# kpham-augment/LongLive

Measured on AMD Instinct MI355X. Metric: generated frames/sec (832x480) LongLive-1.3B, frame-sink + short-window attention, 4 denoise steps + clean-context pass, higher is better.
Workload: dtype bf16

## Files before the change

### include/longlive_hip.h

```cpp
#ifndef LONGLIVE_HIP_H
#define LONGLIVE_HIP_H

#include <stdint.h>

#ifdef __cplusplus
extern "C" {
#endif

typedef uint16_t ll_bf16;
typedef void* ll_stream;

enum ll_status {
  LL_OK = 0,
  LL_ERR_INVALID_ARG = -1,
  LL_ERR_LAUNCH = -2,
  LL_ERR_UNSUPPORTED = -3
};

enum ll_epilogue {
  LL_EPI_BIAS = 0,
  LL_EPI_BIAS_GELU = 1,
  LL_EPI_BIAS_GATE_RES = 2,
  LL_EPI_BIAS_RES = 3
};
// ... 68 lines not shown
               const ll_bf16* mod, int nmod, int gate_idx, int rows_per_batch, int frame_len, ll_stream stream);
int ll_gemm_mx_qkv(const uint8_t* xq, const uint8_t* sx, const uint8_t* wq, const uint8_t* sw, const ll_bf16* bias, ll_bf16* out,
                   int M, int N, int K, int ldo, ll_bf16* cache_v, int B, int L, int S, int write_start, int roped_offset,
                   int write_len, ll_stream stream);
int ll_ln_modulate_mx(const ll_bf16* x, uint8_t* q, uint8_t* qs, const ll_bf16* e, const ll_bf16* mod, int nmod, int shift_idx,
                      int scale_idx, int B, int L, int C, int F, float eps, ll_stream stream);
int ll_ln_modulate_tab_mx(const ll_bf16* x, uint8_t* q, uint8_t* qs, const float* tab, int nmod, int shift_idx, int scale_idx,
                          int B, int L, int C, int F, float eps, ll_stream stream);
int ll_layernorm_affine_mx(const ll_bf16* x, const ll_bf16* w, const ll_bf16* b, uint8_t* q, uint8_t* qs, int rows, int C,
                           float eps, ll_stream stream);
int ll_gemm_plan_mx(int M, int N, int K, char* out, int cap);

int ll_quantize_mx6(const ll_bf16* x, uint8_t* q, uint8_t* qs, int rows, int K, int ldx, ll_stream stream);
int ll_gemm_mx6(const uint8_t* xq, const uint8_t* sx, const uint8_t* wq, const uint8_t* sw, const ll_bf16* bias, ll_bf16* out,
                uint8_t* q_out, uint8_t* s_out, int M, int N, int K, int ldo, int epilogue, const ll_bf16* res, const ll_bf16* e,
                const ll_bf16* mod, int nmod, int gate_idx, int rows_per_batch, int frame_len, ll_stream stream);
int ll_gemm_mx6_qkv(const uint8_t* xq, const uint8_t* sx, const uint8_t* wq, const uint8_t* sw, const ll_bf16* bias, ll_bf16* out,
                    int M, int N, int K, int ldo, ll_bf16* cache_v, int B, int L, int S, int write_start, int roped_offset,
                    int write_len, ll_stream stream);
int ll_ln_modulate_mx6(const ll_bf16* x, uint8_t* q, uint8_t* qs, const ll_bf16* e, const ll_bf16* mod, int nmod, int shift_idx,
                       int scale_idx, int B, int L, int C, int F, float eps, ll_stream stream);
int ll_ln_modulate_tab_mx6(const ll_bf16* x, uint8_t* q, uint8_t* qs, const float* tab, int nmod, int shift_idx, int scale_idx,
                           int B, int L, int C, int F, float eps, ll_stream stream);
int ll_layernorm_affine_mx6(const ll_bf16* x, const ll_bf16* w, const ll_bf16* b, uint8_t* q, uint8_t* qs, int rows, int C,
                            float eps, ll_stream stream);
int ll_gemm_plan_mx6(int M, int N, int K, char* out, int cap);

int ll_quantize_mx4(const ll_bf16* x, uint8_t* q, uint8_t* qs, int rows, int K, int ldx, ll_stream stream);
int ll_gemm_mx4w6(const uint8_t* xq, const uint8_t* sx, const uint8_t* wq, const uint8_t* sw, const ll_bf16* bias, ll_bf16* out,
                  uint8_t* q_out, uint8_t* s_out, int M, int N, int K, int ldo, int epilogue, const ll_bf16* res, const ll_bf16* e,
                  const ll_bf16* mod, int nmod, int gate_idx, int rows_per_batch, int frame_len, ll_stream stream);
int ll_gemm_mx4w6_qkv(const uint8_t* xq, const uint8_t* sx, const uint8_t* wq, const uint8_t* sw, const ll_bf16* bias, ll_bf16* out,
                      int M, int N, int K, int ldo, ll_bf16* cache_v, int B, int L, int S, int write_start, int roped_offset,
                      int write_len, ll_stream stream);
int ll_gemm_plan_mx4w6(int M, int N, int K, char* out, int cap);

int ll_gemm_mx4(const uint8_t* xq, const uint8_t* sx, const uint8_t* wq, const uint8_t* sw, const ll_bf16* bias, ll_bf16* out,
                uint8_t* q_out, uint8_t* s_out, int M, int N, int K, int ldo, int epilogue, const ll_bf16* res, const ll_bf16* e,
                const ll_bf16* mod, int nmod, int gate_idx, int rows_per_batch, int frame_len, ll_stream stream);
int ll_gemm_mx4_qkv(const uint8_t* xq, const uint8_t* sx, const uint8_t* wq, const uint8_t* sw, const ll_bf16* bias, ll_bf16* out,
                    int M, int N, int K, int ldo, ll_bf16* cache_v, int B, int L, int S, int write_start, int roped_offset,
                    int write_len, ll_stream stream);
int ll_ln_modulate_mx4(const ll_bf16* x, uint8_t* q, uint8_t* qs, const ll_bf16* e, const ll_bf16* mod, int nmod, int shift_idx,
                       int scale_idx, int B, int L, int C, int F, float eps, ll_stream stream);
int ll_ln_modulate_tab_mx4(const ll_bf16* x, uint8_t* q, uint8_t* qs, const float* tab, int nmod, int shift_idx, int scale_idx,
                           int B, int L, int C, int F, float eps, ll_stream stream);
int ll_layernorm_affine_mx4(const ll_bf16* x, const ll_bf16* w, const ll_bf16* b, uint8_t* q, uint8_t* qs, int rows, int C,
                            float eps, ll_stream stream);
int ll_gemm_plan_mx4(int M, int N, int K, char* out, int cap);

int ll_quantize_rows_f8(const ll_bf16* x, uint8_t* q, float* scale, int rows, int K, int ldx, ll_stream stream);
int ll_gemm_f8(const uint8_t* xq, const float* sx, const uint8_t* wq, const float* sw, const ll_bf16* bias, ll_bf16* out,
               int M, int N, int K, int ldo, int epilogue, const ll_bf16* res, const ll_bf16* e, const ll_bf16* mod,
               int nmod, int gate_idx, int rows_per_batch, int frame_len, ll_stream stream);
int ll_gemm_f8_qkv(const uint8_t* xq, const float* sx, const uint8_t* wq, const float* sw, const ll_bf16* bias, ll_bf16* out,
                   int M, int N, int K, int ldo, ll_bf16* cache_v, int B, int L, int S, int write_start, int roped_offset,
                   int write_len, ll_stream stream);
int ll_ln_modulate_f8(const ll_bf16* x, uint8_t* q, float* qscale, const ll_bf16* e, const ll_bf16* mod, int nmod, int shift_idx,
                      int scale_idx, int B, int L, int C, int F, float eps, ll_stream stream);
int ll_ln_modulate_tab_f8(const ll_bf16* x, uint8_t* q, float* qscale, const float* tab, int nmod, int shift_idx, int scale_idx,
                          int B, int L, int C, int F, float eps, ll_stream stream);
int ll_layernorm_affine_f8(const ll_bf16* x, const ll_bf16* w, const ll_bf16* b, uint8_t* q, float* qscale, int rows, int C,
                           float eps, ll_stream stream);
int ll_gemm_plan_f8(int M, int N, int K, char* out, int cap);

int ll_kv_shadow_mx(const ll_bf16* k, const ll_bf16* v, uint8_t* kq, uint8_t* ks, uint8_t* vq, uint8_t* vs, int B, int S, int S32, int H,
                    int head_dim, int lo, int hi, ll_stream stream);
int ll_flash_attn_mx(const ll_bf16* q, const uint8_t* kq, const uint8_t* ks, const uint8_t* vq, const uint8_t* vs, ll_bf16* out, int B,
                     int Lq, int H, int head_dim, int ldq, int ldo, int S, int S32, int seg0_start, int seg0_len, int seg1_start,
                     int seg1_len, float scale, ll_stream stream);
int ll_flash_attn_mx_plan(int Lq, int H, int B, int seg0_start, int seg0_len, int seg1_start, int seg1_len, char* out, int cap);

int ll_linear_small(const ll_bf16* x, const ll_bf16* w, const ll_bf16* bias, ll_bf16* out, int M, int N, int K,
                    int act_in, int act_out, ll_stream stream);

int ll_flash_attn(const ll_bf16* q, const ll_bf16* k, const ll_bf16* v, ll_bf16* out, int B, int Lq, int H, int ldq,
                  int ldo, int ldk, long long k_batch_stride, int seg0_start, int seg0_len, int seg1_start,
                  int seg1_len, float scale, ll_stream stream);

int ll_gemm_ssq_planes(int M, int N, int K);
int ll_gemm_bf16_ssq(const ll_bf16* x, const ll_bf16* w, const ll_bf16* bias, ll_bf16* out, float* ssq, int M, int N, int K, int ldx,
                     int ldo, ll_stream stream);
int ll_flash_attn_qnorm_ok(int H, int nkeys);
int ll_flash_attn_qnorm(const ll_bf16* q, const float* ssq, const ll_bf16* norm_w, float eps, const ll_bf16* k, const ll_bf16* v,
                        ll_bf16* out, int B, int Lq, int H, int ldq, int ldo, int ldk, long long k_batch_stride, int key_start,
                        int nkeys, float scale, ll_stream stream);


int ll_patchify(const ll_bf16* x, ll_bf16* patches, int B, int F, int Cin, int H, int W, ll_stream stream);

int ll_sinusoid(const float* t, ll_bf16* out, int n, int dim, ll_stream stream);

int ll_unpatchify_x0(const ll_bf16* head, const ll_bf16* xt, const float* sigma, ll_bf16* flow, ll_bf16* x0, int B,
                     int F, int Cout, int H, int W, ll_stream stream);

int ll_add_noise(const ll_bf16* x0, const ll_bf16* noise, const float* sigma, ll_bf16* out, int N, long long inner,
                 ll_stream stream);

int ll_sigma_lookup(const float* t, const float* timesteps, const float* sigmas, float* out, int n, int n_table,
                    ll_stream stream);

int ll_synth_hash(float* out, long long lo, long long n, unsigned long long stream_const, int kind, ll_stream stream);


int ll_conv_cl(const ll_bf16* x, const ll_bf16* zero16, const ll_bf16* w, const ll_bf16* bias, const ll_bf16* res,
               ll_bf16* out, int T, int H, int W, int Cin, int Cout, int Kpad, int KT, int KH, int upsample, int ldo,
               ll_stream stream);
int ll_conv_cl_rms_ok(int H, int W, int Cin, int Cout, int KT, int KH, int upsample);
int ll_conv_cl_rms(const ll_bf16* x, const ll_bf16* zero16, const ll_bf16* w, const ll_bf16* bias, const ll_bf16* res, ll_bf16* out,
                   const ll_bf16* rms_gamma, ll_bf16* out_rms, int rms_silu, int T, int H, int W, int Cin, int Cout, int Kpad, int KT,
                   int KH, int upsample, int ldo, ll_stream stream);

int ll_rms_silu_cl(const ll_bf16* x, const ll_bf16* gamma, ll_bf16* out, long long pixels, int C, int do_silu,
                   ll_stream stream);

int ll_softmax_rows(const ll_bf16* s, ll_bf16* p, int rows, int N, int ld, float scale, ll_stream stream);

int ll_vae_unscale_cl(const ll_bf16* z, const ll_bf16* mean, const ll_bf16* inv_std, ll_bf16* out, int T, int C, int h,
                      int w, ll_stream stream);

int ll_cl_to_tchw_clamp(const ll_bf16* x, float* out, int T, int H, int W, int ldc, ll_stream stream);


int ll_t5_rmsnorm(const ll_bf16* x, const ll_bf16* w, ll_bf16* out, int rows, int C, float eps, ll_stream stream);

int ll_t5_gated_gelu(const ll_bf16* h, ll_bf16* out, long long M, int F, ll_stream stream);

int ll_gather_rows(const ll_bf16* table, const long long* ids, ll_bf16* out, int n, int C, long long vocab, ll_stream stream);

int ll_t5_attention(const ll_bf16* q, const ll_bf16* k, const ll_bf16* vt, const ll_bf16* bias_tab, ll_bf16* out, int L,
                    int H, int ldqk, int ldo, int seq_len, ll_stream stream);

#ifdef __cplusplus
}
#endif
#endif
```

### longlive_amd/_lib.py

```python
from __future__ import annotations

import ctypes as C
import os

_HERE = os.path.dirname(os.path.abspath(__file__))
LIB_PATH = os.path.join(_HERE, "liblonglive_hip.so")

ABI_VERSION = 111

_p, _i, _f, _ll = C.c_void_p, C.c_int, C.c_float, C.c_longlong

SIGNATURES = {
    "ll_version": [],
    "ll_last_error": [],
    "ll_set_tuning": [C.c_char_p, _i],
    "ll_gemm_plan": [_i, _i, _i, _i, C.c_char_p, _i],
    "ll_gemm_plan_epi": [_i, _i, _i, _i, _i, _i, C.c_char_p, _i],
    "ll_flash_attn_plan": [_i, _i, _i, _i, _i, _i, C.c_char_p, _i],
    "ll_ln_modulate": [_p, _p, _p, _p, _i, _i, _i, _i, _i, _i, _i, _f, _p],
    "ll_modulation_table": [_p, _p, _p, _i, _i, _i, _i, _p],
    "ll_modulation_table_f32": [_p, _p, _p, _i, _i, _i, _i, C.c_uint, _p],
    "ll_ln_modulate_tab": [_p, _p, _p, _p, _p, _i, _i, _i, _i, _i, _i, _i, _f, _p],
    "ll_layernorm_affine": [_p, _p, _p, _p, _i, _i, _f, _p],
    "ll_ln_modulate_q8": [_p, _p, _p, _p, _p, _i, _i, _i, _i, _i, _i, _i, _f, _p],
    "ll_layernorm_affine_q8": [_p, _p, _p, _p, _p, _i, _i, _f, _p],
    "ll_rmsnorm": [_p, _p, _p, _i, _i, _i, _i, _f, _p],
    "ll_qk_norm_rope_kv_store": [_p, _p, _p, _p, _p, _p, _p, _p, _i, _i, _i, _i, _i, _i, _i, _i, _i, _i, _f, _p],
    "ll_kv_roll": [_p, _p, _i, _i, _i, _i, _i, _i, _p],
    "ll_gemm_bf16": [_p, _p, _p, _p, _i, _i, _i, _i, _i, _i, _p, _p, _p, _i, _i, _i, _i, _p],
    "ll_gemm_ksplit_plan": [_i, _i, _i],
    "ll_gemm_ksplit_workspace_bytes": [_i, _i, _i],
    "ll_gemm_bf16_ksplit": [_p, _p, _p, _p, _i, _i, _i, _i, _i, _i, _p, _p, _ll, _p],
    "ll_gemm_bf16_ksplit_t5norm": [_p, _p, _p, _p, _i, _i, _i, _i, _i, _p, _p, _f, _p, _p, _ll, _p],
    "ll_gemm_w8a8": [_p, _p, _p, _p, _p, _p, _i, _i, _i, _i, _i, _p, _p, _p, _i, _i, _i, _i, _p],
    "ll_gemm_bf16_qkv": [_p, _p, _p, _p, _i, _i, _i, _i, _i, _p, _i, _i, _i, _i, _i, _i, _p],
    "ll_gemm_w8a8_qkv": [_p, _p, _p, _p, _p, _p, _i, _i, _i, _i, _p, _i, _i, _i, _i, _i, _i, _p],
    "ll_quantize_rows": [_p, _p, _p, _i, _i, _i, _p],
    "ll_linear_small": [_p, _p, _p, _p, _i, _i, _i, _i, _i, _p],
    "ll_flash_attn": [_p, _p, _p, _p, _i, _i, _i, _i, _i, _i, _ll, _i, _i, _i, _i, _f, _p],
    "ll_patchify": [_p, _p, _i, _i, _i, _i, _i, _p],
    "ll_sinusoid": [_p, _p, _i, _i, _p],
    "ll_unpatchify_x0": [_p, _p, _p, _p, _p, _i, _i, _i, _i, _i, _p],
    "ll_add_noise": [_p, _p, _p, _p, _i, _ll, _p],
    "ll_sigma_lookup": [_p, _p, _p, _p, _i, _i, _p],
    "ll_synth_hash": [_p, _ll, _ll, C.c_ulonglong, _i, _p],
    "ll_gemm_ssq_planes": [_i, _i, _i],
    "ll_gemm_bf16_ssq": [_p, _p, _p, _p, _p, _i, _i, _i, _i, _i, _p],
    "ll_flash_attn_qnorm_ok": [_i, _i],
    "ll_flash_attn_qnorm": [_p, _p, _p, _f, _p, _p, _p, _i, _i, _i, _i, _i, _i, _ll, _i, _i, _f, _p],
    "ll_conv_cl": [_p] * 6 + [_i] * 10 + [_p],
    "ll_conv_cl_rms_ok": [_i] * 7,
    "ll_conv_cl_rms": [_p] * 8 + [_i] * 11 + [_p],
    "ll_rms_silu_cl": [_p, _p, _p, _ll, _i, _i, _p],
    "ll_softmax_rows": [_p, _p, _i, _i, _i, _f, _p],
    "ll_vae_unscale_cl": [_p, _p, _p, _p, _i, _i, _i, _i, _p],
    "ll_cl_to_tchw_clamp": [_p, _p, _i, _i, _i, _i, _p],
    "ll_t5_rmsnorm": [_p, _p, _p, _i, _i, _f, _p],
    "ll_t5_gated_gelu": [_p, _p, _ll, _i, _p],
    "ll_gather_rows": [_p, _p, _p, _i, _i, _ll, _p],
    "ll_t5_attention": [_p, _p, _p, _p, _p, _i, _i, _i, _i, _i, _p],
    "ll_quantize_mx": [_p, _p, _p, _i, _i, _i, _p],
    "ll_gemm_mx": [_p, _p, _p, _p, _p, _p, _p, _p, _i, _i, _i, _i, _i, _p, _p, _p, _i, _i, _i, _i, _p],
    "ll_gemm_mx_qkv": [_p, _p, _p, _p, _p, _p, _i, _i, _i, _i, _p, _i, _i, _i, _i, _i, _i, _p],
    "ll_ln_modulate_mx": [_p, _p, _p, _p, _p, _i, _i, _i, _i, _i, _i, _i, _f, _p],
    "ll_ln_modulate_tab_mx": [_p, _p, _p, _p, _i, _i, _i, _i, _i, _i, _i, _f, _p],
    "ll_layernorm_affine_mx": [_p, _p, _p, _p, _p, _i, _i, _f, _p],
    "ll_gemm_plan_mx": [_i, _i, _i, C.c_char_p, _i],
    "ll_kv_shadow_mx": [_p] * 6 + [_i] * 7 + [_p],
    "ll_flash_attn_mx": [_p] * 6 + [_i] * 12 + [_f, _p],
    "ll_flash_attn_mx_plan": [_i] * 7 + [C.c_char_p, _i],
    "ll_quantize_rows_f8": [_p, _p, _p, _i, _i, _i, _p],
    "ll_gemm_f8": [_p, _p, _p, _p, _p, _p, _i, _i, _i, _i, _i, _p, _p, _p, _i, _i, _i, _i, _p],
    "ll_gemm_f8_qkv": [_p, _p, _p, _p, _p, _p, _i, _i, _i, _i, _p, _i, _i, _i, _i, _i, _i, _p],
    "ll_ln_modulate_f8": [_p, _p, _p, _p, _p, _i, _i, _i, _i, _i, _i, _i, _f, _p],
    "ll_ln_modulate_tab_f8": [_p, _p, _p, _p, _i, _i, _i, _i, _i, _i, _i, _f, _p],
    "ll_layernorm_affine_f8": [_p, _p, _p, _p, _p, _i, _i, _f, _p],
    "ll_gemm_plan_f8": [_i, _i, _i, C.c_char_p, _i],
    "ll_quantize_mx6": [_p, _p, _p, _i, _i, _i, _p],
    "ll_gemm_mx6": [_p] * 8 + [_i] * 5 + [_p] * 3 + [_i] * 4 + [_p],
    "ll_gemm_mx6_qkv": [_p] * 6 + [_i] * 4 + [_p] + [_i] * 6 + [_p],
    "ll_ln_modulate_mx6": [_p] * 5 + [_i] * 7 + [_f, _p],
    "ll_ln_modulate_tab_mx6": [_p] * 4 + [_i] * 7 + [_f, _p],
    "ll_layernorm_affine_mx6": [_p] * 5 + [_i, _i, _f, _p],
    "ll_gemm_plan_mx6": [_i, _i, _i, C.c_char_p, _i],
    "ll_quantize_mx4": [_p, _p, _p, _i, _i, _i, _p],
    "ll_gemm_mx4w6": [_p] * 8 + [_i] * 5 + [_p] * 3 + [_i] * 4 + [_p],
    "ll_gemm_mx4w6_qkv": [_p] * 6 + [_i] * 4 + [_p] + [_i] * 6 + [_p],
    "ll_gemm_plan_mx4w6": [_i, _i, _i, C.c_char_p, _i],
    "ll_gemm_mx4": [_p] * 8 + [_i] * 5 + [_p] * 3 + [_i] * 4 + [_p],
    "ll_gemm_mx4_qkv": [_p] * 6 + [_i] * 4 + [_p] + [_i] * 6 + [_p],
    "ll_ln_modulate_mx4": [_p] * 5 + [_i] * 7 + [_f, _p],
    "ll_ln_modulate_tab_mx4": [_p] * 4 + [_i] * 7 + [_f, _p],
    "ll_layernorm_affine_mx4": [_p] * 5 + [_i, _i, _f, _p],
    "ll_gemm_plan_mx4": [_i, _i, _i, C.c_char_p, _i],
}
_RESTYPES = {"ll_last_error": C.c_char_p, "ll_gemm_ksplit_workspace_bytes": C.c_longlong}

_lib = None


def load() -> C.CDLL:
    global _lib
    if _lib is not None:
        return _lib
    path = os.environ.get("LONGLIVE_HIP_LIB", LIB_PATH)
    if not os.path.exists(path):
        raise RuntimeError(
            f"{path} not found: the HIP extension is not built (make -C longlive_amd/csrc). "
            "longlive_amd has no CPU fallback by design.")
    lib = C.CDLL(path)
    for name, argtypes in SIGNATURES.items():
        try:
            fn = getattr(lib, name)
        except AttributeError as exc:
            raise RuntimeError(f"{LIB_PATH} does not export {name}") from exc
        fn.argtypes = argtypes
        fn.restype = _RESTYPES.get(name, C.c_int)
    if lib.ll_version() != ABI_VERSION:
        raise RuntimeError(f"{path} has ABI version {lib.ll_version()}, this binding needs {ABI_VERSION}: rebuild it "
                           "(make -C longlive_amd/csrc); a stale library would misread every argument list")
    _lib = lib
    for kv in filter(None, os.environ.get("LL_TUNING", "").split(",")):
        k, v = kv.split("=")
        if lib.ll_set_tuning(k.encode(), int(v)) != 0:
            raise RuntimeError(f"LL_TUNING: {lib.ll_last_error().decode()}")
    return lib


def check(rc: int, what: str = "") -> None:
    if rc != 0:
        msg = load().ll_last_error()
# ... 2 lines not shown
```

### longlive_amd/csrc/elementwise.hip

```cpp
#include "common.h"
#include "mx.h"
#include "mx4.h"
#include "mx6.h"

#define MAXCH 4

struct RowRegs {
  f32x2 p[MAXCH][4];
};
struct RowWords {
  unsigned w[MAXCH][4];
};

template <bool FULL>
__device__ __forceinline__ bool in_row(int c, int C) {
  return FULL || c < C;
}

template <int NCH, bool FULL>
__device__ __forceinline__ void load_words(const bf16* __restrict__ p, int C, int lane, RowWords& r) {
#pragma unroll
  for (int i = 0; i < NCH; ++i) {
    int c = (lane + 64 * i) * 8;
    uint4 t = make_uint4(0u, 0u, 0u, 0u);
// ... 866 lines not shown

#define DISPATCH_NCH(C, CALL)                                              \
  do {                                                                     \
    int nch_ = ((C) + 511) / 512;                                          \
    bool full_ = ((C) % 512) == 0;                                         \
    if (nch_ == 1) { if (full_) CALL(1, true); else CALL(1, false); }      \
    else if (nch_ == 2) { if (full_) CALL(2, true); else CALL(2, false); } \
    else if (nch_ == 3) { if (full_) CALL(3, true); else CALL(3, false); } \
    else { if (full_) CALL(4, true); else CALL(4, false); }                \
  } while (0)

static inline bool row_ok(int C) { return C > 0 && C <= 2048 && (C % 8) == 0; }

static int ln_modulate_launch(const ll_bf16* x, ll_bf16* out, int8_t* q, float* qscale, const ll_bf16* e,
                              const ll_bf16* mod, int nmod, int shift_idx, int scale_idx, int B, int L, int C, int F,
                              float eps, ll_stream stream, bool f8 = false) {
  LL_REQUIRE(row_ok(C), "ll_ln_modulate: C=%d must be a multiple of 8 and <= 2048", C);
  LL_REQUIRE(F > 0 && L % F == 0, "ll_ln_modulate: L=%d not divisible by F=%d", L, F);
  LL_REQUIRE(shift_idx >= 0 && shift_idx < nmod && scale_idx >= 0 && scale_idx < nmod, "ll_ln_modulate: bad mod index");
  int rows = B * L;
  if (rows == 0) return LL_OK;
  dim3 grid((rows + 3) / 4);
#define CALL2(N, FL, F8)                                                                                                     \
  do {                                                                                                                   \
    if (mod)                                                                                                             \
      hipLaunchKernelGGL((ln_modulate_kernel<N, FL, false, F8>), grid, dim3(256), 0, (hipStream_t)stream, (const bf16*)x, (bf16*)out, \
                         (const bf16*)e, (const bf16*)mod, nmod, shift_idx, scale_idx, rows, L, C, L / F, F, eps, q, qscale); \
    else                                                                                                                 \
      hipLaunchKernelGGL((ln_modulate_kernel<N, FL, true, F8>), grid, dim3(256), 0, (hipStream_t)stream, (const bf16*)x, (bf16*)out,  \
                         (const bf16*)e, (const bf16*)mod, nmod, shift_idx, scale_idx, rows, L, C, L / F, F, eps, q, qscale); \
  } while (0)
#define CALL(N, FL) CALL2(N, FL, false)
#define CALL_F8(N, FL) CALL2(N, FL, true)
  if (f8) DISPATCH_NCH(C, CALL_F8);
  else DISPATCH_NCH(C, CALL);
#undef CALL
#undef CALL_F8
#undef CALL2
  return ll_check_launch("ll_ln_modulate");
}

extern "C" int ll_modulation_table(const ll_bf16* e, const ll_bf16* mods, ll_bf16* out, int num_layers, int BF, int nmod, int C,
                                   ll_stream stream) {
  LL_REQUIRE(C > 0 && C % 8 == 0 && nmod > 0 && num_layers >= 0 && BF >= 0, "ll_modulation_table: bad shape");
  long long chunks = (long long)num_layers * BF * nmod * (C / 8);
  if (chunks == 0) return LL_OK;
  LL_REQUIRE(chunks < (1LL << 31) * 256, "ll_modulation_table: too large");
  hipLaunchKernelGGL(modulation_table_kernel, dim3((unsigned)((chunks + 255) / 256)), dim3(256), 0, (hipStream_t)stream,
                     (const bf16*)e, (const bf16*)mods, (bf16*)out, num_layers, BF, nmod * (C / 8));
  return ll_check_launch("ll_modulation_table");
}

extern "C" int ll_ln_modulate(const ll_bf16* x, ll_bf16* out, const ll_bf16* e, const ll_bf16* mod, int nmod,
                              int shift_idx, int scale_idx, int B, int L, int C, int F, float eps, ll_stream stream) {
  return ln_modulate_launch(x, out, nullptr, nullptr, e, mod, nmod, shift_idx, scale_idx, B, L, C, F, eps, stream);
}

extern "C" int ll_ln_modulate_q8(const ll_bf16* x, int8_t* q, float* qscale, const ll_bf16* e, const ll_bf16* mod,
                                 int nmod, int shift_idx, int scale_idx, int B, int L, int C, int F, float eps,
                                 ll_stream stream) {
  LL_REQUIRE(q && qscale, "ll_ln_modulate_q8: q and qscale are required");
  return ln_modulate_launch(x, nullptr, q, qscale, e, mod, nmod, shift_idx, scale_idx, B, L, C, F, eps, stream);
}

extern "C" int ll_ln_modulate_f8(const ll_bf16* x, uint8_t* q, float* qscale, const ll_bf16* e, const ll_bf16* mod, int nmod,
                                 int shift_idx, int scale_idx, int B, int L, int C, int F, float eps, ll_stream stream) {
  LL_REQUIRE(x != nullptr && e != nullptr, "ll_ln_modulate_f8: x and e are required");
  LL_REQUIRE(q && qscale, "ll_ln_modulate_f8: codes and scales are required");
  return ln_modulate_launch(x, nullptr, (int8_t*)q, qscale, e, mod, nmod, shift_idx, scale_idx, B, L, C, F, eps, stream, true);
}

extern "C" int ll_modulation_table_f32(const ll_bf16* e, const ll_bf16* mods, float* out, int num_layers, int BF, int nmod, int C,
                                       unsigned one_plus_mask, ll_stream stream) {
  LL_REQUIRE(C > 0 && C % 8 == 0 && nmod > 0 && nmod <= 32 && num_layers >= 0 && BF >= 0, "ll_modulation_table_f32: bad shape");
  LL_REQUIRE(nmod == 32 || (one_plus_mask >> nmod) == 0, "ll_modulation_table_f32: one_plus_mask names a chunk >= nmod=%d", nmod);
  long long chunks = (long long)num_layers * BF * nmod * (C / 8);
  if (chunks == 0) return LL_OK;
  LL_REQUIRE(chunks < (1LL << 31) * 256, "ll_modulation_table_f32: too large");
  hipLaunchKernelGGL(modulation_table_f32_kernel, dim3((unsigned)((chunks + 255) / 256)), dim3(256), 0, (hipStream_t)stream,
                     (const bf16*)e, (const bf16*)mods, out, num_layers, BF, nmod, C / 8, one_plus_mask);
  return ll_check_launch("ll_modulation_table_f32");
}

extern "C" int ll_ln_modulate_tab(const ll_bf16* x, ll_bf16* out, int8_t* q, float* qscale, const float* tab, int nmod,
                                  int shift_idx, int scale_idx, int B, int L, int C, int F, float eps, ll_stream stream) {
  LL_REQUIRE(row_ok(C), "ll_ln_modulate_tab: C=%d must be a multiple of 8 and <= 2048", C);
  LL_REQUIRE(F > 0 && L % F == 0, "ll_ln_modulate_tab: L=%d not divisible by F=%d", L, F);
  LL_REQUIRE(shift_idx >= 0 && shift_idx < nmod && scale_idx >= 0 && scale_idx < nmod, "ll_ln_modulate_tab: bad mod index");
  LL_REQUIRE((out != nullptr) != (q != nullptr), "ll_ln_modulate_tab: exactly one of out (bf16) and q (int8, with qscale) is required");
  LL_REQUIRE(q == nullptr || qscale != nullptr, "ll_ln_modulate_tab: q needs qscale");
  int rows = B * L;
  if (rows == 0) return LL_OK;
  dim3 grid((rows + 3) / 4);
#define CALL(N, FL)                                                                                                      \
  hipLaunchKernelGGL((ln_modulate_tab_kernel<N, FL>), grid, dim3(256), 0, (hipStream_t)stream, (const bf16*)x, (bf16*)out, tab, \
                     nmod, shift_idx, scale_idx, rows, L, C, L / F, F, eps, q, qscale)
  DISPATCH_NCH(C, CALL);
#undef CALL
  return ll_check_launch("ll_ln_modulate_tab");
}

extern "C" int ll_ln_modulate_tab_f8(const ll_bf16* x, uint8_t* q, float* qscale, const float* tab, int nmod, int shift_idx, int scale_idx,
                                     int B, int L, int C, int F, float eps, ll_stream stream) {
  LL_REQUIRE(x != nullptr && tab != nullptr, "ll_ln_modulate_tab_f8: x and tab are required");
  LL_REQUIRE(q && qscale, "ll_ln_modulate_tab_f8: codes and scales are required");
  LL_REQUIRE(row_ok(C), "ll_ln_modulate_tab_f8: C=%d must be a multiple of 8 and <= 2048", C);
  LL_REQUIRE(F > 0 && L % F == 0, "ll_ln_modulate_tab_f8: L=%d not divisible by F=%d", L, F);
  LL_REQUIRE(shift_idx >= 0 && shift_idx < nmod && scale_idx >= 0 && scale_idx < nmod, "ll_ln_modulate_tab_f8: bad mod index");
  int rows = B * L;
  if (rows == 0) return LL_OK;
  dim3 grid((rows + 3) / 4);
#define CALL(N, FL)                                                                                                           \
  hipLaunchKernelGGL((ln_modulate_tab_kernel<N, FL, true>), grid, dim3(256), 0, (hipStream_t)stream, (const bf16*)x, (bf16*)nullptr, \
                     tab, nmod, shift_idx, scale_idx, rows, L, C, L / F, F, eps, (int8_t*)q, qscale)
  DISPATCH_NCH(C, CALL);
#undef CALL
  return ll_check_launch("ll_ln_modulate_tab_f8");
}

static int layernorm_affine_launch(const ll_bf16* x, const ll_bf16* w, const ll_bf16* b, ll_bf16* out, int8_t* q,
                                   float* qscale, int rows, int C, float eps, ll_stream stream, bool f8 = false) {
  LL_REQUIRE(row_ok(C), "ll_layernorm_affine: C=%d must be a multiple of 8 and <= 2048", C);
  if (rows == 0) return LL_OK;
  dim3 grid((rows + 3) / 4);
#define CALL2(N, FL, F8)                                                                                         \
  hipLaunchKernelGGL((layernorm_affine_kernel<N, FL, F8>), grid, dim3(256), 0, (hipStream_t)stream, (const bf16*)x, \
                     (const bf16*)w, (const bf16*)b, (bf16*)out, rows, C, eps, q, qscale)
#define CALL(N, FL) CALL2(N, FL, false)
#define CALL_F8(N, FL) CALL2(N, FL, true)
  if (f8) DISPATCH_NCH(C, CALL_F8);
  else DISPATCH_NCH(C, CALL);
#undef CALL
#undef CALL_F8
#undef CALL2
  return ll_check_launch("ll_layernorm_affine");
}

extern "C" int ll_layernorm_affine(const ll_bf16* x, const ll_bf16* w, const ll_bf16* b, ll_bf16* out, int rows, int C,
                                   float eps, ll_stream stream) {
  return layernorm_affine_launch(x, w, b, out, nullptr, nullptr, rows, C, eps, stream);
}

extern "C" int ll_layernorm_affine_q8(const ll_bf16* x, const ll_bf16* w, const ll_bf16* b, int8_t* q, float* qscale,
                                      int rows, int C, float eps, ll_stream stream) {
  LL_REQUIRE(q && qscale, "ll_layernorm_affine_q8: q and qscale are required");
  return layernorm_affine_launch(x, w, b, nullptr, q, qscale, rows, C, eps, stream);
}

extern "C" int ll_layernorm_affine_f8(const ll_bf16* x, const ll_bf16* w, const ll_bf16* b, uint8_t* q, float* qscale, int rows, int C,
                                      float eps, ll_stream stream) {
  LL_REQUIRE(x != nullptr && w != nullptr && b != nullptr, "ll_layernorm_affine_f8: x, w and b are required");
  LL_REQUIRE(q && qscale, "ll_layernorm_affine_f8: codes and scales are required");
  return layernorm_affine_launch(x, w, b, nullptr, (int8_t*)q, qscale, rows, C, eps, stream, true);
}

static int mx_row_ok(const char* fn, int C, const void* q, const void* qs) {
  LL_REQUIRE(C > 0 && C <= 2048 && C % MX_BLOCK == 0, "%s: C=%d must be a multiple of 32 and <= 2048", fn, C);
  LL_REQUIRE(q != nullptr && qs != nullptr, "%s: codes and scales are required", fn);
  return LL_OK;
}

extern "C" int ll_ln_modulate_mx(const ll_bf16* x, uint8_t* q, uint8_t* qs, const ll_bf16* e, const ll_bf16* mod, int nmod,
                                 int shift_idx, int scale_idx, int B, int L, int C, int F, float eps, ll_stream stream) {
  if (int rc = mx_row_ok("ll_ln_modulate_mx", C, q, qs)) return rc;
  LL_REQUIRE(x != nullptr && e != nullptr, "ll_ln_modulate_mx: x and e are required");
  LL_REQUIRE(F > 0 && L % F == 0, "ll_ln_modulate_mx: L=%d not divisible by F=%d", L, F);
// ... 294 lines not shown
```

### longlive_amd/csrc/gemm.hip

```cpp
#include <stdio.h>
#include <string.h>
#include <atomic>

#include "gemm_common.h"
#include "mx.h"

#define V2_BM 256
#define V2_STAGE ((V2_BM + BN) * ROWB)

template <int EPI, int Q>
__global__ __launch_bounds__(512, 2) void gemm_kernel_v2(const char* __restrict__ X, const char* __restrict__ Wt,
                                                         bf16* __restrict__ Y, int M, int N, int nk, size_t xrow_bytes,
                                                         size_t wrow_bytes, int ldo, int ntm, int ntn, int gm, int lds_epi, EpiArgs ea) {
  extern __shared__ __attribute__((aligned(16))) char smem[];
  typedef typename Ty<Q>::frag frag_t;
  const int tid = threadIdx.x, lane = tid & 63;
  const int wave = __builtin_amdgcn_readfirstlane(tid >> 6);
  const int wm = wave >> 1, wn = wave & 1;
  int lid = xcd_remap(blockIdx.x, ntm * ntn), mt_, nt_;
  tile_of(lid, ntm, ntn, gm, mt_, nt_);
  const int m0 = mt_ * V2_BM, n0 = nt_ * BN;

  typename Ty<Q>::acc acc[4][4];
#pragma unroll
// ... 490 lines not shown
    if (v5 || v6) {                                                                                                    \
      (void)ll_lds_attr((const void*)gemm_kernel_v5<E, Q, 2, 4, 8, 3>, 2 * (256 + 192) * ROWB);                       \
      (void)ll_lds_attr((const void*)gemm_kernel_v5<E, Q, 4, 2, 4, 7>, 2 * (256 + 224) * ROWB);                       \
      if (v5)                                                                                                          \
        hipLaunchKernelGGL((gemm_kernel_v5<E, Q, 2, 4, 8, 3>), grid, block, lds, s, (const char*)x, (const char*)w, out, M, N, nk, \
                           xrow_bytes, wrow_bytes, ldo, ntm, ntn, gm, lds_epi, ea);                                                 \
      else                                                                                                             \
        hipLaunchKernelGGL((gemm_kernel_v5<E, Q, 4, 2, 4, 7>), grid, block, lds, s, (const char*)x, (const char*)w, out, M, N, nk, \
                           xrow_bytes, wrow_bytes, ldo, ntm, ntn, gm, lds_epi, ea);                                                 \
    } else if (v3) {                                                                                                   \
      (void)ll_lds_attr((const void*)gemm_kernel_v3<E, Q>, (int)lds);                                                 \
      hipLaunchKernelGGL((gemm_kernel_v3<E, Q>), grid, block, lds, s, (const char*)x, (const char*)w, out, M, N, nk,   \
                         xrow_bytes, wrow_bytes, ldo, ntm, ntn, gm, lds_epi, ea);                                      \
    } else {                                                                                                           \
      (void)ll_lds_attr((const void*)gemm_kernel_v2<E, Q>, (int)lds);                                          \
      hipLaunchKernelGGL((gemm_kernel_v2<E, Q>), grid, block, lds, s, (const char*)x, (const char*)w, out, M, N, nk, \
                         xrow_bytes, wrow_bytes, ldo, ntm, ntn, gm, lds_epi, ea);                                      \
    }                                                                                                                  \
  } while (0)
  switch (epilogue) {
    case LL_EPI_BIAS: LAUNCH(LL_EPI_BIAS); break;
    case LL_EPI_BIAS_GELU: LAUNCH(LL_EPI_BIAS_GELU); break;
    case LL_EPI_BIAS_GATE_RES: LAUNCH(LL_EPI_BIAS_GATE_RES); break;
    default: LAUNCH(LL_EPI_BIAS_RES); break;
  }
#undef LAUNCH
  return LL_OK;
}

static int check_epilogue(const char* fn, int M, int N, int ldo, int epilogue, const void* bias, const void* res,
                          const void* e, const void* mod, int nmod, int gate_idx, int rows_per_batch, int frame_len) {
  LL_REQUIRE(N > 0 && N % 8 == 0, "%s: N=%d must be a positive multiple of 8", fn, N);
  LL_REQUIRE(ldo >= N && ldo % 4 == 0, "%s: ldo=%d must be >= N and a multiple of 4", fn, ldo);
  LL_REQUIRE(bias != nullptr, "%s: bias is required", fn);
  LL_REQUIRE(epilogue >= 0 && epilogue <= 3, "%s: unknown epilogue %d", fn, epilogue);
  if (epilogue == LL_EPI_BIAS_GATE_RES) {
    LL_REQUIRE(res && e, "%s: gate-residual epilogue needs res and e (mod may be NULL: e then holds bf16(mod + e))", fn);
    LL_REQUIRE(frame_len > 0 && rows_per_batch > 0 && rows_per_batch % frame_len == 0 && M % rows_per_batch == 0,
               "%s: rows_per_batch=%d / frame_len=%d do not tile M=%d", fn, rows_per_batch, frame_len, M);
    LL_REQUIRE(gate_idx >= 0 && gate_idx < nmod, "%s: gate_idx %d outside nmod %d", fn, gate_idx, nmod);
  }
  if (epilogue == LL_EPI_BIAS_RES) LL_REQUIRE(res != nullptr, "%s: residual epilogue needs res", fn);
  return LL_OK;
}

extern "C" int ll_gemm_bf16(const ll_bf16* x, const ll_bf16* w, const ll_bf16* bias, ll_bf16* out, int M, int N, int K,
                            int ldx, int ldo, int epilogue, const ll_bf16* res, const ll_bf16* e, const ll_bf16* mod,
                            int nmod, int gate_idx, int rows_per_batch, int frame_len, ll_stream stream) {
  LL_REQUIRE(K > 0 && K % 64 == 0, "ll_gemm_bf16: K=%d must be a positive multiple of 64", K);
  LL_REQUIRE(ldx >= K && ldx % 8 == 0, "ll_gemm_bf16: ldx=%d must be >= K and a multiple of 8", ldx);
  int rc = check_epilogue("ll_gemm_bf16", M, N, ldo, epilogue, bias, res, e, mod, nmod, gate_idx, rows_per_batch, frame_len);
  if (rc) return rc;
  if (M == 0) return LL_OK;
  EpiArgs ea{(const bf16*)bias, (const bf16*)res, (const bf16*)e, (const bf16*)mod, nullptr, nullptr, nmod, gate_idx,
             rows_per_batch, frame_len, frame_len > 0 && rows_per_batch > 0 ? rows_per_batch / frame_len : 0};
  if (int lrc = launch_gemm<GQ_BF16>(x, w, (bf16*)out, M, N, K, (size_t)ldx * 2, (size_t)K * 2, ldo, epilogue, ea, (hipStream_t)stream)) return lrc;
  return ll_check_launch("ll_gemm_bf16");
}

static int device_cus();
int gemm_asm_ssq_launch(const bf16* x, const bf16* w, const bf16* bias, bf16* out, float* ssq, int M, int N, int K, int ldx, int ldo, int gm,
                        hipStream_t s);
extern "C" int ll_gemm_ssq_planes(int M, int N, int K) {
  if (!gemm_asm_wanted(LL_EPI_BIAS)) return 0;
  return gemm_asm_width(M, N, K, K, LL_EPI_BIAS, true, false, false, 0) == 128 && N / 128 <= 16 ? N / 128 : 0;
}
extern "C" int ll_gemm_bf16_ssq(const ll_bf16* x, const ll_bf16* w, const ll_bf16* bias, ll_bf16* out, float* ssq, int M, int N, int K,
                                int ldx, int ldo, ll_stream stream) {
  LL_REQUIRE(K > 0 && K % 64 == 0, "ll_gemm_bf16_ssq: K=%d must be a positive multiple of 64", K);
  LL_REQUIRE(ldx >= K && ldx % 8 == 0, "ll_gemm_bf16_ssq: ldx=%d must be >= K and a multiple of 8", ldx);
  int rc = check_epilogue("ll_gemm_bf16_ssq", M, N, ldo, LL_EPI_BIAS, bias, nullptr, nullptr, nullptr, 0, 0, 0, 0);
  if (rc) return rc;
  LL_REQUIRE(ssq != nullptr && ((size_t)ssq & 3) == 0, "ll_gemm_bf16_ssq: ssq is required");
  LL_REQUIRE(ll_gemm_ssq_planes(M, N, K) > 0 && ldx == K, "ll_gemm_bf16_ssq: %d x %d x %d is not covered by the generated kernel under the current "
             "tuning (ask ll_gemm_ssq_planes first and run ll_gemm_bf16 + ll_rmsnorm instead)", M, N, K);
  if (M == 0) return LL_OK;
  const int r = gemm_asm_ssq_launch((const bf16*)x, (const bf16*)w, (const bf16*)bias, (bf16*)out, ssq, M, N, K, ldx, ldo, g_gemm_group_m,
                                    (hipStream_t)stream);
  if (r < 0) return r;
  LL_REQUIRE(r == 1, "ll_gemm_bf16_ssq: the generated kernel refused a shape its plan accepted");
  return ll_check_launch("ll_gemm_bf16_ssq");
}

extern "C" int ll_gemm_ksplit_plan(int M, int N, int K) {
  if (!gemm_asm_wanted(LL_EPI_BIAS)) return 0;
  return gemm_ksplit_splits(M, N, K, device_cus());
}
extern "C" long long ll_gemm_ksplit_workspace_bytes(int M, int N, int K) {
  const int S = ll_gemm_ksplit_plan(M, N, K);
  return S ? (long long)S * M * N * 4 : 0;
}
extern "C" int ll_gemm_bf16_ksplit(const ll_bf16* x, const ll_bf16* w, const ll_bf16* bias, ll_bf16* out, int M, int N, int K,
                                   int ldx, int ldo, int epilogue, const ll_bf16* res, void* workspace,
                                   long long workspace_bytes, ll_stream stream) {
  LL_REQUIRE(K > 0 && K % 64 == 0, "ll_gemm_bf16_ksplit: K=%d must be a positive multiple of 64", K);
  LL_REQUIRE(ldx >= K && ldx % 8 == 0, "ll_gemm_bf16_ksplit: ldx=%d must be >= K and a multiple of 8", ldx);
  LL_REQUIRE(epilogue == LL_EPI_BIAS || epilogue == LL_EPI_BIAS_RES, "ll_gemm_bf16_ksplit: epilogue %d (bias or bias + residual only)", epilogue);
  int rc = check_epilogue("ll_gemm_bf16_ksplit", M, N, ldo, epilogue, bias, res, nullptr, nullptr, 0, 0, 0, 0);
  if (rc) return rc;
  LL_REQUIRE(workspace_bytes >= 0 && (workspace != nullptr || workspace_bytes == 0), "ll_gemm_bf16_ksplit: workspace_bytes without a workspace");
  if (M == 0) return LL_OK;
  const int S = ll_gemm_ksplit_plan(M, N, K);
  if (S >= 2 && workspace != nullptr && ldo % 8 == 0) {
    LL_REQUIRE(workspace_bytes >= (long long)S * M * N * 4 && ((size_t)workspace & 15) == 0,
               "ll_gemm_bf16_ksplit: workspace of %lld bytes, need %lld (16-byte aligned)", workspace_bytes, (long long)S * M * N * 4);
    const int r = gemm_asm_ksplit_launch((const bf16*)x, (const bf16*)w, (const bf16*)bias, (bf16*)out, M, N, K, ldx, ldo, epilogue,
                                         (const bf16*)res, (float*)workspace, S, g_gemm_group_m, (hipStream_t)stream, nullptr, 0.f, nullptr);
    if (r) return r < 0 ? r : ll_check_launch("ll_gemm_bf16_ksplit");
  }
  EpiArgs ea{(const bf16*)bias, (const bf16*)res, nullptr, nullptr, nullptr, nullptr, 0, 0, 0, 0, 0};
  if (int lrc = launch_gemm<GQ_BF16>(x, w, (bf16*)out, M, N, K, (size_t)ldx * 2, (size_t)K * 2, ldo, epilogue, ea, (hipStream_t)stream)) return lrc;
  return ll_check_launch("ll_gemm_bf16_ksplit");
}

extern "C" int ll_gemm_bf16_ksplit_t5norm(const ll_bf16* x, const ll_bf16* w, const ll_bf16* bias, ll_bf16* out, int M, int N, int K,
                                          int ldx, int ldo, const ll_bf16* res, const ll_bf16* norm_w, float eps, ll_bf16* h_out,
                                          void* workspace, long long workspace_bytes, ll_stream stream) {
  LL_REQUIRE(K > 0 && K % 64 == 0, "ll_gemm_bf16_ksplit_t5norm: K=%d must be a positive multiple of 64", K);
  LL_REQUIRE(ldx >= K && ldx % 8 == 0, "ll_gemm_bf16_ksplit_t5norm: ldx=%d must be >= K and a multiple of 8", ldx);
  LL_REQUIRE(norm_w != nullptr && h_out != nullptr, "ll_gemm_bf16_ksplit_t5norm: needs the norm weight and an output for the normalised rows");
  LL_REQUIRE(ldo == N, "ll_gemm_bf16_ksplit_t5norm: ldo=%d must equal N=%d (the norm runs over whole rows)", ldo, N);
  int rc = check_epilogue("ll_gemm_bf16_ksplit_t5norm", M, N, ldo, LL_EPI_BIAS_RES, bias, res, nullptr, nullptr, 0, 0, 0, 0);
  if (rc) return rc;
  LL_REQUIRE(workspace_bytes >= 0 && (workspace != nullptr || workspace_bytes == 0), "ll_gemm_bf16_ksplit_t5norm: workspace_bytes without a workspace");
  if (M == 0) return LL_OK;
  const int S = ll_gemm_ksplit_plan(M, N, K);
  if (S >= 2 && workspace != nullptr && N <= 4096) {
    LL_REQUIRE(workspace_bytes >= (long long)S * M * N * 4 && ((size_t)workspace & 15) == 0,
               "ll_gemm_bf16_ksplit_t5norm: workspace of %lld bytes, need %lld (16-byte aligned)", workspace_bytes, (long long)S * M * N * 4);
    const int r = gemm_asm_ksplit_launch((const bf16*)x, (const bf16*)w, (const bf16*)bias, (bf16*)out, M, N, K, ldx, ldo, LL_EPI_BIAS_RES,
                                         (const bf16*)res, (float*)workspace, S, g_gemm_group_m, (hipStream_t)stream, (const bf16*)norm_w, eps,
                                         (bf16*)h_out);
    if (r) return r < 0 ? r : ll_check_launch("ll_gemm_bf16_ksplit_t5norm");
  }
  rc = ll_gemm_bf16_ksplit(x, w, bias, out, M, N, K, ldx, ldo, LL_EPI_BIAS_RES, res, workspace, workspace_bytes, stream);
  if (rc) return rc;
  return ll_t5_rmsnorm(out, norm_w, h_out, M, N, eps, stream);
}

static int device_cus() {
  static int cus[64];
  int dev = 0;
  if (hipGetDevice(&dev) != hipSuccess || dev < 0 || dev >= 64) return 0;
  if (cus[dev] == 0) {
    int n = 0;
    if (hipDeviceGetAttribute(&n, hipDeviceAttributeMultiprocessorCount, dev) != hipSuccess) n = 0;
    cus[dev] = n > 0 ? n : -1;
  }
  return cus[dev] > 0 ? cus[dev] : 0;
}

extern "C" int ll_gemm_plan_epi(int M, int N, int K, int int8, int epilogue, int plain, char* out, int cap) {
  LL_REQUIRE(out != nullptr && cap > 0, "ll_gemm_plan_epi: needs an output buffer");
  if (!int8 && gemm_asm_wanted(epilogue)) {
    const int wn = gemm_asm_width(M, N, K, K, epilogue, plain != 0, plain == 2, plain == 2 && (2 * (N / 3)) % 192 == 0, 1);
    if (wn) { gemm_asm_plan(M, N, wn, epilogue, out, cap, false); ll_plan_append_knobs(out, cap); return LL_OK; }
  }
  if (int8 && (g_gemm_asm & 16) && gemm_asm_wanted(epilogue)) {
    const int wn = gemm_asm_width_i8(M, N, K, epilogue, plain != 0, plain == 2, plain == 2 && (2 * (N / 3)) % 192 == 0, 1);
    if (wn) { gemm_asm_plan(M, N, wn, epilogue, out, cap, true); ll_plan_append_knobs(out, cap); return LL_OK; }
  }
  return ll_gemm_plan(M, N, K, int8, out, cap);
}

extern "C" int ll_gemm_w8a8(const int8_t* xq, const float* sx, const int8_t* wq, const float* sw, const ll_bf16* bias,
                            ll_bf16* out, int M, int N, int K, int ldo, int epilogue, const ll_bf16* res,
// ... 134 lines not shown
```

### longlive_amd/csrc/gemm_asm.hip

```cpp
#include "gemm_common.h"

#define GA_NAME gemm_asm_224_gelu
#define GA_WN 224
#define GA_INC "build/gemm_asm_224_1.inc"
#include "gemm_asm_kernel.inl"
#undef GA_NAME
#undef GA_WN
#undef GA_INC
#define GA_NAME gemm_asm_256_bias
#define GA_WN 256
#define GA_INC "build/gemm_asm_256_0.inc"
#include "gemm_asm_kernel.inl"
#undef GA_NAME
#undef GA_WN
#undef GA_INC
#define GA_NAME gemm_asm_192_bias
#define GA_WN 192
#define GA_INC "build/gemm_asm_192_0.inc"
#include "gemm_asm_kernel.inl"
#undef GA_NAME
#undef GA_WN
#undef GA_INC
#define GA_NAME gemm_asm_128_bias
#define GA_WN 128
#define GA_INC "build/gemm_asm_128_0.inc"
#include "gemm_asm_kernel.inl"
#undef GA_NAME
#undef GA_WN
#undef GA_INC
#define GA_NAME gemm_asm_128_gate_res
#define GA_WN 128
#define GA_INC "build/gemm_asm_128_2.inc"
#include "gemm_asm_kernel.inl"
#undef GA_NAME
#undef GA_WN
#undef GA_INC
#define GA_NAME gemm_asm_128_res
#define GA_WN 128
#define GA_INC "build/gemm_asm_128_3.inc"
#include "gemm_asm_kernel.inl"
#undef GA_NAME
#undef GA_WN
#undef GA_INC

#define GA_NAME gemm_asmp_224_gelu
#define GA_INC "build/gemm_asmp_224_1.inc"
#include "gemm_asm_kernel_p.inl"
#undef GA_NAME
#undef GA_INC
#define GA_NAME gemm_asmp_192_bias
#define GA_INC "build/gemm_asmp_192_0.inc"
#include "gemm_asm_kernel_p.inl"
#undef GA_NAME
#undef GA_INC
#define GA_NAME gemm_asmp_128_bias
#define GA_INC "build/gemm_asmp_128_0.inc"
#include "gemm_asm_kernel_p.inl"
#undef GA_NAME
#undef GA_INC
#define GA_NAME gemm_asmp_128_gate_res
#define GA_INC "build/gemm_asmp_128_2.inc"
#include "gemm_asm_kernel_p.inl"
#undef GA_NAME
#undef GA_INC
#define GA_NAME gemm_asmp_128_res
#define GA_INC "build/gemm_asmp_128_3.inc"
#include "gemm_asm_kernel_p.inl"
#undef GA_NAME
#undef GA_INC

#define GA_NAME gemm_asm_128_bias_ssq
#define GA_WN 128
#define GA_INC "build/gemm_asm_128_5.inc"
#define GA_SSQ 1
#include "gemm_asm_kernel.inl"
#undef GA_SSQ
#undef GA_NAME
#undef GA_WN
#undef GA_INC

#define GA_NAME gemm_asm_128_partial
#define GA_WN 128
#define GA_INC "build/gemm_asm_128_4.inc"
#define GA_PARTIAL 1
#include "gemm_asm_kernel.inl"
#undef GA_PARTIAL
#undef GA_NAME
#undef GA_WN
#undef GA_INC

#define GA_NAME gemm_asmq_224_gelu
#define GA_WN 224
#define GA_INC "build/gemm_asmq_224_1.inc"
#define GA_I8 1
#include "gemm_asm_kernel.inl"
#undef GA_I8
#undef GA_NAME
#undef GA_WN
#undef GA_INC
#define GA_NAME gemm_asmq_192_bias
#define GA_WN 192
#define GA_INC "build/gemm_asmq_192_0.inc"
#define GA_I8 1
#include "gemm_asm_kernel.inl"
#undef GA_I8
#undef GA_NAME
#undef GA_WN
#undef GA_INC
#define GA_NAME gemm_asmq_128_bias
#define GA_WN 128
#define GA_INC "build/gemm_asmq_128_0.inc"
#define GA_I8 1
#include "gemm_asm_kernel.inl"
#undef GA_I8
#undef GA_NAME
#undef GA_WN
#undef GA_INC
#define GA_NAME gemm_asmq_128_gate_res
#define GA_WN 128
#define GA_INC "build/gemm_asmq_128_2.inc"
#define GA_I8 1
#include "gemm_asm_kernel.inl"
#undef GA_I8
#undef GA_NAME
#undef GA_WN
#undef GA_INC
#define GA_NAME gemm_asmq_128_res
#define GA_WN 128
#define GA_INC "build/gemm_asmq_128_3.inc"
#define GA_I8 1
#include "gemm_asm_kernel.inl"
#undef GA_I8
#undef GA_NAME
#undef GA_WN
#undef GA_INC

int g_gemm_asm_persistent = 1;
static int gemm_asm_cus() {
  static int cus[64];
  int dev = 0;
  if (hipGetDevice(&dev) != hipSuccess || dev < 0 || dev >= 64) return 0;
  if (cus[dev] == 0) {
    int n = 0;
    if (hipDeviceGetAttribute(&n, hipDeviceAttributeMultiprocessorCount, dev) != hipSuccess) n = 0;
    cus[dev] = n > 0 ? n : -1;
  }
  return cus[dev] > 0 ? cus[dev] : 0;
}

int gemm_asm_width(int M, int N, int K, int ldx, int epilogue, bool plain, bool has_v, bool v_ok, int frame_len) {
  if (!plain || M <= 0 || K % 64 != 0 || K < 256 || (ldx % 8) != 0) return 0;
  if (epilogue == LL_EPI_BIAS_GATE_RES && frame_len <= 0) return 0;
  if ((long long)256 * ldx * 2 >= 0x7fffffffLL || (long long)256 * K * 2 >= 0x7fffffffLL) return 0;
  if (has_v) return (v_ok && epilogue == LL_EPI_BIAS && N % 192 == 0) ? 192 : 0;
  if (epilogue == LL_EPI_BIAS_GELU) return N % 224 == 0 ? 224 : 0;
  if (epilogue == LL_EPI_BIAS && N > 2048 && N % 192 == 0) return 192;
  if (epilogue == LL_EPI_BIAS && M <= 1024 && N >= 16384 && N % 256 == 0) return 256;
  if (N % 128 == 0 && (N <= 2048 || M <= 1024) &&
      (epilogue == LL_EPI_BIAS || epilogue == LL_EPI_BIAS_GATE_RES || epilogue == LL_EPI_BIAS_RES)) return 128;
  return 0;
}

int gemm_asm_launch(const bf16* x, const bf16* w, bf16* out, int M, int N, int K, int ldx, int ldo, int epilogue, const EpiArgs& ea,
                    int gm, hipStream_t s) {
  const bool has_v = ea.v_out != nullptr;
  const bool v_ok = has_v && ea.v_L == M && ea.v_col0 % 192 == 0 && ea.v_C > 0;
  const int wn = gemm_asm_width(M, N, K, ldx, epilogue, ea.sx == nullptr && ea.mod == nullptr, has_v, v_ok, ea.frame_len);
  if (!wn) return 0;
  const void* fn = wn == 224 ? (const void*)gemm_asm_224_gelu
                   : wn == 256 ? (const void*)gemm_asm_256_bias
                   : wn == 192 ? (const void*)gemm_asm_192_bias
                   : epilogue == LL_EPI_BIAS ? (const void*)gemm_asm_128_bias
                   : epilogue == LL_EPI_BIAS_GATE_RES ? (const void*)gemm_asm_128_gate_res : (const void*)gemm_asm_128_res;
  const int lds = 3 * wn * 128 + 4 * 2 * 8192;
  const int ntm = (M + 255) / 256, ntn = N / wn;
  const int cus = gemm_asm_cus() & ~7;
  const void* pfn = wn == 224 ? (const void*)gemm_asmp_224_gelu
                    : wn == 192 ? (const void*)gemm_asmp_192_bias
                    : wn != 128 ? nullptr
                    : epilogue == LL_EPI_BIAS ? (const void*)gemm_asmp_128_bias
                    : epilogue == LL_EPI_BIAS_GATE_RES ? (const void*)gemm_asmp_128_gate_res : (const void*)gemm_asmp_128_res;
  const bool persistent = g_gemm_asm_persistent && pfn != nullptr && cus >= 8 && ntm * ntn > cus;
  if (persistent) fn = pfn;
  if (int rc = ll_lds_attr(fn, lds)) return rc;
  const bf16* gate = epilogue == LL_EPI_BIAS_GATE_RES ? ea.e + (size_t)ea.gate_idx * N : nullptr;
  const int gstride = ea.nmod * N * 2;
  bf16* v_out = ea.v_out;
  int v_col0 = ea.v_col0, v_C = ea.v_C, v_shift = ea.v_write_start - ea.v_roped_offset, v_lo = ea.v_roped_offset,
      v_hi = ea.v_roped_offset + ea.v_write_len;
  void* args[] = {(void*)&x, (void*)&w, (void*)&ea.bias, (void*)&out, (void*)&ea.res, (void*)&gate, (void*)&M, (void*)&N, (void*)&K,
                  (void*)&ldx, (void*)&ldo, (void*)&ea.frame_len, (void*)&gstride, (void*)&ntm, (void*)&ntn, (void*)&gm,
                  (void*)&v_out, (void*)&v_col0, (void*)&v_C, (void*)&v_shift, (void*)&v_lo, (void*)&v_hi};
  if (hipLaunchKernel(fn, dim3(persistent ? cus : ntm * ntn), dim3(256), args, (size_t)lds, s) != hipSuccess) return ll_check_launch("gemm_asm");
  return 1;
}

int gemm_asm_ssq_launch(const bf16* x, const bf16* w, const bf16* bias, bf16* out, float* ssq, int M, int N, int K, int ldx, int ldo, int gm,
                        hipStream_t s) {
  if (gemm_asm_width(M, N, K, ldx, LL_EPI_BIAS, true, false, false, 0) != 128) return 0;
  const void* fn = (const void*)gemm_asm_128_bias_ssq;
  const int lds = 3 * 128 * 128 + 4 * 2 * 8192;
  if (int rc = ll_lds_attr(fn, lds)) return rc;
  const int ntm = (M + 255) / 256, ntn = N / 128;
  const bf16* nullb = nullptr;
  bf16* nov = nullptr;
  int zero = 0;
  void* args[] = {(void*)&x, (void*)&w, (void*)&bias, (void*)&out, (void*)&nullb, (void*)&nullb, (void*)&M, (void*)&N, (void*)&K,
                  (void*)&ldx, (void*)&ldo, (void*)&zero, (void*)&zero, (void*)&ntm, (void*)&ntn, (void*)&gm,
                  (void*)&nov, (void*)&zero, (void*)&zero, (void*)&zero, (void*)&zero, (void*)&zero, (void*)&ssq};
  if (hipLaunchKernel(fn, dim3(ntm * ntn), dim3(256), args, (size_t)lds, s) != hipSuccess) return ll_check_launch("gemm_asm_128_bias_ssq");
  return 1;
}

const char* gemm_asm_plan(int M, int N, int wn, int epilogue, char* out, int cap, bool i8) {
  const char* tail = wn == 224 ? "gelu" : wn == 256 ? "bias" : epilogue == LL_EPI_BIAS ? "bias" : epilogue == LL_EPI_BIAS_GATE_RES ? "gate_res" : "res";
  const int tiles = ((M + 255) / 256) * (N / wn), cus = gemm_asm_cus() & ~7;
  if (!i8 && g_gemm_asm_persistent && wn != 256 && cus >= 8 && tiles > cus)
    snprintf(out, (size_t)cap, "gemm_asmp_%d_%s<bf16> tile 256x%d (4 waves x 64 rows, one wave per SIMD, generated schedule), %d persistent workgroups "
             "walk %d tiles, next tile staged under the epilogue", wn, tail, wn, cus, tiles);
  else
    snprintf(out, (size_t)cap, "gemm_asm%s_%d_%s<%s> tile 256x%d (4 waves x 64 rows, one wave per SIMD, generated schedule), %d workgroups", i8 ? "q" : "", wn,
             tail, i8 ? "i8" : "bf16", wn, tiles);
  return out;
}

int gemm_asm_width_i8(int M, int N, int K, int epilogue, bool plain, bool has_v, bool v_ok, int frame_len) {
  if (!plain || M <= 0 || K % 128 != 0 || K < 512 || (long long)256 * K >= 0x7fffffffLL) return 0;
  if (epilogue == LL_EPI_BIAS_GATE_RES && frame_len <= 0) return 0;
  if (has_v) return (v_ok && epilogue == LL_EPI_BIAS && N % 192 == 0) ? 192 : 0;
  if (epilogue == LL_EPI_BIAS_GELU) return N % 224 == 0 ? 224 : 0;
  if (epilogue == LL_EPI_BIAS && N > 2048 && N % 192 == 0) return 192;
  if (N % 128 == 0 && N <= 2048) return 128;
  return 0;
}

template <int EPI>
__global__ __launch_bounds__(256) void gemm_ksplit_reduce_kernel(const float* __restrict__ part, int splits, int M, int N,
                                                                 const bf16* __restrict__ bias, const bf16* __restrict__ res,
                                                                 bf16* __restrict__ out, int ldo) {
  const int n8 = N / 8;
  const long long idx = (long long)blockIdx.x * 256 + threadIdx.x;
  if (idx >= (long long)M * n8) return;
  const int m = (int)(idx / n8), n = (int)(idx - (long long)m * n8) * 8;
  float acc[8];
#pragma unroll
  for (int j = 0; j < 8; ++j) acc[j] = 0.f;
  for (int s = 0; s < splits; ++s) {
    const float4* p = reinterpret_cast<const float4*>(part + ((size_t)s * M + m) * N + n);
    float4 a = p[0], b = p[1];
    acc[0] += a.x; acc[1] += a.y; acc[2] += a.z; acc[3] += a.w; acc[4] += b.x; acc[5] += b.y; acc[6] += b.z; acc[7] += b.w;
  }
  bf16x8 bv = *reinterpret_cast<const bf16x8*>(bias + n), o;
  bf16x8 rv;
  if (EPI == LL_EPI_BIAS_RES) rv = *reinterpret_cast<const bf16x8*>(res + (size_t)m * ldo + n);
#pragma unroll
  for (int j = 0; j < 8; ++j) {
    bf16 v = (bf16)(acc[j] + (float)bv[j]);
    o[j] = EPI == LL_EPI_BIAS_RES ? (bf16)((float)rv[j] + (float)v) : v;
  }
  *reinterpret_cast<bf16x8*>(out + (size_t)m * ldo + n) = o;
}

__global__ __launch_bounds__(256) void gemm_ksplit_reduce_norm_kernel(const float* __restrict__ part, int splits, int M, int N,
                                                                      const bf16* __restrict__ bias, const bf16* __restrict__ res,
                                                                      bf16* __restrict__ out, int ldo, const bf16* __restrict__ nw,
                                                                      float eps, bf16* __restrict__ h_out) {
  __shared__ float sh[4];
  const int m = blockIdx.x;
  bf16x8 xn[2];
  float ss = 0.f;
#pragma unroll
  for (int i = 0; i < 2; ++i) {
    const int n = threadIdx.x * 8 + 2048 * i;
    if (n < N) {
      float acc[8];
#pragma unroll
      for (int j = 0; j < 8; ++j) acc[j] = 0.f;
      for (int s = 0; s < splits; ++s) {
        const float4* p = reinterpret_cast<const float4*>(part + ((size_t)s * M + m) * N + n);
        float4 a = p[0], b = p[1];
        acc[0] += a.x; acc[1] += a.y; acc[2] += a.z; acc[3] += a.w; acc[4] += b.x; acc[5] += b.y; acc[6] += b.z; acc[7] += b.w;
      }
      bf16x8 bv = *reinterpret_cast<const bf16x8*>(bias + n), rv = *reinterpret_cast<const bf16x8*>(res + (size_t)m * ldo + n), o;
#pragma unroll
      for (int j = 0; j < 8; ++j) {
        bf16 v = (bf16)(acc[j] + (float)bv[j]);
        o[j] = (bf16)((float)rv[j] + (float)v);
        ss += (float)o[j] * (float)o[j];
      }
      xn[i] = o;
      *reinterpret_cast<bf16x8*>(out + (size_t)m * ldo + n) = o;
    }
  }
  ss = t5_block_sum(ss, sh);
  const float r = rsqrtf(ss / (float)N + eps);
#pragma unroll
// ... 79 lines not shown
```

### longlive_amd/csrc/gen/gemm_asm_gen.py

```python
#!/usr/bin/env python3
from __future__ import annotations

import os
import sys

sys.path.insert(0, os.path.dirname(os.path.abspath(__file__)))
import attn_asm_gen as _A
from attn_asm_gen import Gen, finalize, lint, sreg, vreg, areg, to_inc, f32bits, spread

EPI_BIAS, EPI_GELU, EPI_GATE_RES, EPI_RES = 0, 1, 2, 3
EPI_PARTIAL = 4
EPI_BIAS_SSQ = 5

S_X, S_W, S_Y, S_BIAS, S_RES, S_GATE = 8, 10, 12, 14, 16, 18
S_LDX, S_LDW, S_LDO = 20, 21, 22
S_ROWS, S_COLS, S_NK = 23, 24, 25
S_FLEN, S_GSTRIDE, S_M0 = 26, 27, 28
S_ROWLO = 29
S_SX, S_SW = 64, 66
S_SSQ = 64
S_XRS, S_WRS = 32, 36
S_WAVE, S_I, S_T0, S_T1, S_T2 = 40, 41, 44, 45, 46
S_WM0, S_XK, S_WK, S_XKMAX, S_WKMAX = 47, 48, 49, 43, 62
S_MSK = 50
V_TID = 0

NSLOT, XU = 3, 2
S_XM0 = 30

S_XB, S_WB, S_YB, S_BIASB, S_RESB, S_GATEB = 84, 86, 88, 90, 92, 94
S_LDO0, S_MM, S_NN = 68, 69, 70
S_TILE, S_GRID, S_NTILES, S_NTM, S_NTN, S_GM = 71, 72, 73, 74, 75, 76
S_VHI, S_VOUT, S_VCOL0, S_VC2, S_VSHIFT, S_VLO = 77, 78, 80, 81, 82, 83
S_XN, S_WN, S_PF, S_ROWSN = 64, 66, 31, 42
S_MT, S_NT = 54, 55


def KN(k):
    return _A.knob_env("ASM_G_", k, 0)


class Cfg:
    def __init__(self, WN, epi, i8=False):
        assert WN % 32 == 0 and 64 <= WN <= 256
        assert not (i8 and epi in (EPI_PARTIAL, EPI_BIAS_SSQ))
        self.WN, self.NB, self.MB, self.epi, self.i8 = WN, WN // 32, 2, epi, i8
        self.nacc = self.MB * self.NB * 16
        self.slotb = WN * 128
        self.npw = WN // 32
        self.xbase = NSLOT * self.slotb
        self.xunit = 64 * 128
        self.lds_bytes = self.xbase + 4 * XU * self.xunit
        assert self.lds_bytes <= 160 * 1024
        self.FW = 0
        self.FX = 2 * self.NB * 2 * 4
        nxt = max(self.FX + 2 * self.MB * 4 * 4, 144)
        self.V_WOFF = nxt
        self.V_XROFF = nxt + 12
        self.V_DW = nxt + 16
        self.V_DX = nxt + 24
        self.V_LANE, self.V_R, self.V_H, self.V_ROW = nxt + 32, nxt + 33, nxt + 34, nxt + 35
        self.V_T = 0
        assert nxt + 37 <= 256, nxt
        self.V_EA = nxt + 37
        top = self.V_EA + 5
        if i8:
            self.V_SX = top + 2
            top += 6
        assert top % 2 == 0, top
        self.nl = {EPI_GATE_RES: 6, EPI_RES: 2}.get(epi, 0)
        self.V_E0 = top
        top += 16 if self.nl else 0
        self.V_SS = top
        top += 4 if epi == EPI_BIAS_SSQ else 0
        self.V_EB = top
        self.early_nb = 0 if epi == EPI_PARTIAL else max(0, min(self.NB, (256 - top) // 8))

    def acc(self, mb, nb):
        return (mb * self.NB + nb) * 16

    def fw(self, p, nb, ks):
        return self.FW + ((p * self.NB + nb) * 2 + ks) * 4

    def fx(self, b, mb, ks4):
        return self.FX + ((b * self.MB + mb) * 4 + ks4) * 4


def mfmas(c: Cfg, h):
    p, b, hf = h & 1, (h >> 1) & 1, h & 1
    out = []
    for ks in range(2):
        for nb in range(c.NB):
            for mb in range(c.MB):
                a = areg(c.acc(mb, nb), 16)
                op = "v_mfma_i32_32x32x32_i8" if c.i8 else "v_mfma_f32_32x32x16_bf16"
                out.append(f"{op} {a}, {vreg(c.fw(p, nb, ks), 4)}, {vreg(c.fx(b, mb, 2 * hf + ks), 4)}, {a}")
    return out


def w_frag_reads(c: Cfg, h):
    slot, hs = (h >> 1) % NSLOT, h & 1
    out = []
    for ks in range(2):
        for nb in range(c.NB):
            off = slot * c.slotb + nb * 4096
            b64, imm = off >> 16, off & 0xFFFF
            out.append(f"ds_read_b128 {vreg(c.fw(h & 1, nb, ks), 4)}, {vreg(c.V_WOFF + 4 * b64 + 2 * hs + ks)} offset:{imm}")
    return out


def x_frag_reads(c: Cfg, s):
    out = []
    for ks4 in range(4):
        for mb in range(c.MB):
            out.append(f"ds_read_b128 {vreg(c.fx(s & 1, mb, ks4), 4)}, {vreg(c.V_XROFF + ks4)} offset:{(s % XU) * c.xunit + mb * 4096}")
    return out


def x_dma(c: Cfg, s):
    out = []
    for i in range(8):
        out.append(f"s_add_u32 m0, {sreg(S_XM0)}, {(s % XU) * c.xunit + 1024 * i}")
        out.append(f"buffer_load_dwordx4 {vreg(c.V_DX + i)}, {sreg(S_XRS, 4)}, {sreg(S_XK)} offen lds")
    out.append(f"s_add_u32 {sreg(S_XK)}, {sreg(S_XK)}, 128")
    out.append(f"s_min_u32 {sreg(S_XK)}, {sreg(S_XK)}, {sreg(S_XKMAX)}")
    return out


def w_dma(c: Cfg, s):
    out = []
    for i in range(c.npw):
        out.append(f"s_add_u32 m0, {sreg(S_WM0)}, {(s % NSLOT) * c.slotb + 1024 * i}")
        out.append(f"buffer_load_dwordx4 {vreg(c.V_DW + i)}, {sreg(S_WRS, 4)}, {sreg(S_WK)} offen lds")
    out.append(f"s_add_u32 {sreg(S_WK)}, {sreg(S_WK)}, 128")
    out.append(f"s_min_u32 {sreg(S_WK)}, {sreg(S_WK)}, {sreg(S_WKMAX)}")
    return out


def drop_loads(ops):
    return [o for o in ops if not o.startswith("buffer_load")]


def udiv(g: Gen, q, num, den, T):
    I = g.I
    I(f"v_cvt_f32_u32 {vreg(T)}, {sreg(num)}")
    I(f"v_cvt_f32_u32 {vreg(T + 1)}, {sreg(den)}")
    I(f"v_rcp_f32 {vreg(T + 1)}, {vreg(T + 1)}")
    I("s_nop 0")
    I(f"v_mul_f32 {vreg(T)}, {vreg(T)}, {vreg(T + 1)}")
    I(f"v_cvt_u32_f32 {vreg(T)}, {vreg(T)}")
    I("s_nop 0")
    I(f"v_readfirstlane_b32 {sreg(q)}, {vreg(T)}")
    I("s_nop 0")
    I(f"s_mul_i32 {sreg(S_T2)}, {sreg(q)}, {sreg(den)}")
    I(f"s_cmp_gt_u32 {sreg(S_T2)}, {sreg(num)}")
    I(f"s_cselect_b32 {sreg(S_T2)}, 1, 0")
    I(f"s_sub_u32 {sreg(q)}, {sreg(q)}, {sreg(S_T2)}")
    I(f"s_mul_i32 {sreg(S_T2)}, {sreg(q)}, {sreg(den)}")
    I(f"s_sub_u32 {sreg(S_T2)}, {sreg(num)}, {sreg(S_T2)}")
# ... 11 lines not shown
    I(f"s_lshr_b32 {sreg(hi)}, {sreg(tile)}, 3")
    I(f"s_add_u32 {sreg(q1)}, {sreg(q)}, 1")
    I(f"s_mul_i32 {sreg(a)}, {sreg(x)}, {sreg(q1)}")
    I(f"s_mul_i32 {sreg(b)}, {sreg(r)}, {sreg(q1)}")
    I(f"s_sub_u32 {sreg(c_)}, {sreg(x)}, {sreg(r)}")
    I(f"s_mul_i32 {sreg(c_)}, {sreg(c_)}, {sreg(q)}")
    I(f"s_add_u32 {sreg(b)}, {sreg(b)}, {sreg(c_)}")
    I(f"s_cmp_lt_u32 {sreg(x)}, {sreg(r)}")
    I(f"s_cselect_b32 {sreg(a)}, {sreg(a)}, {sreg(b)}")
    I(f"s_add_u32 {sreg(S_T0)}, {sreg(a)}, {sreg(hi)}")
    I(f"s_mul_i32 {sreg(S_T1)}, {sreg(S_GM)}, {sreg(S_NTN)}")
    udiv(g, 56, S_T0, S_T1, T)
    I(f"s_mul_i32 {sreg(57)}, {sreg(56)}, {sreg(S_T1)}")
    I(f"s_sub_u32 {sreg(S_T0)}, {sreg(S_T0)}, {sreg(57)}")
    I(f"s_mul_i32 {sreg(58)}, {sreg(56)}, {sreg(S_GM)}")
    I(f"s_sub_u32 {sreg(S_T1)}, {sreg(S_NTM)}, {sreg(58)}")
    I(f"s_min_u32 {sreg(S_T1)}, {sreg(S_T1)}, {sreg(S_GM)}")
    udiv(g, S_NT, S_T0, S_T1, T)
    I(f"s_mul_i32 {sreg(57)}, {sreg(S_NT)}, {sreg(S_T1)}")
    I(f"s_sub_u32 {sreg(57)}, {sreg(S_T0)}, {sreg(57)}")
    I(f"s_add_u32 {sreg(S_MT)}, {sreg(58)}, {sreg(57)}")


def add64(g: Gen, dst, base, lo, hi=None):
    g.I(f"s_add_u32 {sreg(dst)}, {sreg(base)}, {sreg(lo)}")
    g.I(f"s_addc_u32 {sreg(dst + 1)}, {sreg(base + 1)}, {sreg(hi) if hi is not None else 0}")


def gen_tile_bases(g: Gen, c, xdst, wdst, rows_dst, skip_label, full: bool, prefix: str):
    I = g.I
    m0r, n0 = 56, 57
    I(f"s_lshl_b32 {sreg(m0r)}, {sreg(S_MT)}, 8")
    I(f"s_mul_i32 {sreg(n0)}, {sreg(S_NT)}, {c.WN}")
    I(f"s_mul_i32 {sreg(S_T0)}, {sreg(m0r)}, {sreg(S_LDX)}")
    I(f"s_mul_hi_u32 {sreg(S_T1)}, {sreg(m0r)}, {sreg(S_LDX)}")
    add64(g, xdst, S_XB, S_T0, S_T1)
    I(f"s_mul_i32 {sreg(S_T0)}, {sreg(n0)}, {sreg(S_LDW)}")
    I(f"s_mul_hi_u32 {sreg(S_T1)}, {sreg(n0)}, {sreg(S_LDW)}")
    add64(g, wdst, S_WB, S_T0, S_T1)
    I(f"s_sub_u32 {sreg(rows_dst)}, {sreg(S_MM)}, {sreg(m0r)}")
    if full:
        I(f"s_sub_u32 {sreg(S_COLS)}, {sreg(S_NN)}, {sreg(n0)}")
        I(f"s_mov_b32 {sreg(S_M0)}, {sreg(m0r)}")
        I(f"s_mov_b32 {sreg(S_ROWLO)}, 0")
        I(f"s_mov_b32 {sreg(S_LDO)}, {sreg(S_LDO0)}")
        I(f"s_lshl_b32 {sreg(58)}, {sreg(n0)}, 1")
        add64(g, S_BIAS, S_BIASB, 58)
        add64(g, S_GATE, S_GATEB, 58)
        I(f"s_mul_i32 {sreg(S_T0)}, {sreg(m0r)}, {sreg(S_LDO0)}")
        I(f"s_mul_hi_u32 {sreg(S_T1)}, {sreg(m0r)}, {sreg(S_LDO0)}")
        I(f"s_add_u32 {sreg(S_T0)}, {sreg(S_T0)}, {sreg(58)}")
        I(f"s_addc_u32 {sreg(S_T1)}, {sreg(S_T1)}, 0")
        add64(g, S_Y, S_YB, S_T0, S_T1)
        add64(g, S_RES, S_RESB, S_T0, S_T1)
    g.uid += 1
    lab = f"{prefix}_NOTV_{g.uid}"
    I(f"s_cmp_eq_u64 {sreg(S_VOUT, 2)}, 0")
    I(f"s_cbranch_scc1 {lab}")
    I(f"s_cmp_lt_u32 {sreg(n0)}, {sreg(S_VCOL0)}")
    I(f"s_cbranch_scc1 {lab}")
    I(f"s_min_i32 {sreg(59)}, {sreg(S_MM)}, {sreg(S_VHI)}")
    I(f"s_sub_i32 {sreg(59)}, {sreg(59)}, {sreg(m0r)}")
    I(f"s_sub_i32 {sreg(60)}, {sreg(S_VLO)}, {sreg(m0r)}")
    I(f"s_max_i32 {sreg(60)}, {sreg(60)}, 0")
    I(f"s_cmp_le_i32 {sreg(59)}, {sreg(60)}")
    I(f"s_cbranch_scc1 {skip_label}")
    I(f"s_mov_b32 {sreg(rows_dst)}, {sreg(59)}")
    if full:
        I(f"s_mov_b32 {sreg(S_ROWLO)}, {sreg(60)}")
        I(f"s_mov_b32 {sreg(S_LDO)}, {sreg(S_VC2)}")
        I(f"s_add_i32 {sreg(S_T2)}, {sreg(m0r)}, {sreg(S_VSHIFT)}")
        I(f"s_mul_i32 {sreg(S_T0)}, {sreg(S_T2)}, {sreg(S_VC2)}")
        I(f"s_mul_hi_i32 {sreg(S_T1)}, {sreg(S_T2)}, {sreg(S_VC2)}")
        I(f"s_sub_u32 {sreg(58)}, {sreg(n0)}, {sreg(S_VCOL0)}")
        I(f"s_lshl_b32 {sreg(58)}, {sreg(58)}, 1")
        I(f"s_add_u32 {sreg(S_T0)}, {sreg(S_T0)}, {sreg(58)}")
        I(f"s_addc_u32 {sreg(S_T1)}, {sreg(S_T1)}, 0")
        add64(g, S_Y, S_VOUT, S_T0, S_T1)
    g.L(lab)


def generate(WN: int, epi: int, prefix: str, i8: bool = False, persistent: bool = False) -> str:
    c = Cfg(WN, epi, i8)
    assert not (persistent and (i8 or epi in (EPI_PARTIAL, EPI_BIAS_SSQ)))
    g = Gen()
    I = g.I
    T = 128
    npw = c.npw
    def ident():
        I(f"v_and_b32 {vreg(c.V_LANE)}, 63, {vreg(V_TID)}")
        I(f"v_lshrrev_b32 {vreg(T)}, 6, {vreg(V_TID)}")
        I("s_nop 0")
        I(f"v_readfirstlane_b32 {sreg(S_WAVE)}, {vreg(T)}")
        I(f"v_and_b32 {vreg(c.V_R)}, 31, {vreg(c.V_LANE)}")
        I(f"v_lshrrev_b32 {vreg(c.V_H)}, 5, {vreg(c.V_LANE)}")
    if persistent:
        ident()
        I(f"s_mov_b32 {sreg(S_PF)}, 0")
        g.L(f"{prefix}_TILE")
        gen_tile_map(g, S_TILE, T)
        gen_tile_bases(g, c, S_X, S_W, S_ROWS, f"{prefix}_NEXT", True, prefix)
    if not persistent:
        ident()
    for rs, base, rows, ld in ((S_XRS, S_X, S_ROWS, S_LDX), (S_WRS, S_W, S_COLS, S_LDW)):
        I(f"s_mov_b32 {sreg(rs)}, {sreg(base)}")
        I(f"s_and_b32 {sreg(rs + 1)}, {sreg(base + 1)}, 0xffff")
        I(f"s_min_u32 {sreg(S_T0)}, {sreg(rows)}, 256")
        I(f"s_mul_i32 {sreg(rs + 2)}, {sreg(S_T0)}, {sreg(ld)}")
        I(f"s_mov_b32 {sreg(rs + 3)}, 0x00020000")
    I(f"s_mov_b32 {sreg(S_XK)}, 0")
    I(f"s_mov_b32 {sreg(S_WK)}, 0")
    I(f"s_lshl_b32 {sreg(S_WKMAX)}, {sreg(S_NK)}, 7")
    I(f"s_sub_u32 {sreg(S_WKMAX)}, {sreg(S_WKMAX)}, 128")
    I(f"s_mov_b32 {sreg(S_XKMAX)}, {sreg(S_WKMAX)}")
    I(f"s_mul_i32 {sreg(S_WM0)}, {sreg(S_WAVE)}, {1024 * npw}")
    I(f"s_mul_i32 {sreg(S_XM0)}, {sreg(S_WAVE)}, {XU * c.xunit}")
    I(f"s_add_u32 {sreg(S_XM0)}, {sreg(S_XM0)}, {c.xbase}")
    I(f"v_lshrrev_b32 {vreg(T)}, 3, {vreg(c.V_LANE)}")
    I(f"v_and_b32 {vreg(T + 1)}, 7, {vreg(c.V_LANE)}")
    for dst, cnt, ld in ((c.V_DW, npw, S_LDW), (c.V_DX, 8, S_LDX)):
        I(f"s_mul_i32 {sreg(S_T0)}, {sreg(S_WAVE)}, {8 * cnt}")
        for i in range(cnt):
            I(f"v_add_u32 {vreg(T + 2)}, {sreg(S_T0)}, {vreg(T)}")
            I(f"v_add_u32 {vreg(T + 2)}, {8 * i}, {vreg(T + 2)}")
            I(f"v_lshrrev_b32 {vreg(T + 3)}, 1, {vreg(T + 2)}")
            I(f"v_and_b32 {vreg(T + 3)}, 7, {vreg(T + 3)}")
            I(f"v_xor_b32 {vreg(T + 3)}, {vreg(T + 3)}, {vreg(T + 1)}")
            I(f"v_lshlrev_b32 {vreg(T + 3)}, 4, {vreg(T + 3)}")
            I(f"v_mul_lo_u32 {vreg(dst + i)}, {vreg(T + 2)}, {sreg(ld)}")
            I(f"v_add_u32 {vreg(dst + i)}, {vreg(dst + i)}, {vreg(T + 3)}")
    I(f"s_lshl_b32 {sreg(S_T0)}, {sreg(S_WAVE)}, 6")
    for mb in range(c.MB):
        I(f"v_add_u32 {vreg(c.V_ROW + mb)}, {sreg(S_T0)}, {vreg(c.V_R)}")
        if mb:
            I(f"v_add_u32 {vreg(c.V_ROW + mb)}, {32 * mb}, {vreg(c.V_ROW + mb)}")
    I(f"v_lshrrev_b32 {vreg(T)}, 1, {vreg(c.V_R)}")
    I(f"v_and_b32 {vreg(T)}, 7, {vreg(T)}")
    I(f"v_lshlrev_b32 {vreg(T + 1)}, 7, {vreg(c.V_R)}")
    for hs in range(2):
        for ks in range(2):
            I(f"v_add_u32 {vreg(T + 2)}, {4 * hs + 2 * ks}, {vreg(c.V_H)}")
            I(f"v_xor_b32 {vreg(T + 2)}, {vreg(T + 2)}, {vreg(T)}")
            I(f"v_lshl_add_u32 {vreg(c.V_WOFF + 2 * hs + ks)}, {vreg(T + 2)}, 4, {vreg(T + 1)}")
            I(f"v_add_u32 {vreg(c.V_WOFF + 4 + 2 * hs + ks)}, 0x10000, {vreg(c.V_WOFF + 2 * hs + ks)}")
            I(f"v_add_u32 {vreg(c.V_WOFF + 8 + 2 * hs + ks)}, 0x20000, {vreg(c.V_WOFF + 2 * hs + ks)}")
            I(f"v_add_u32 {vreg(c.V_XROFF + 2 * hs + ks)}, {sreg(S_XM0)}, {vreg(c.V_WOFF + 2 * hs + ks)}")
    I(f"s_cmp_ge_u32 {sreg(S_T0)}, {sreg(S_ROWS)}")
    I(f"s_cbranch_scc1 {prefix}_IDLE")
    n_early = gen_epilogue_setup(g, c)
    if persistent:
        I(f"s_cmp_eq_u32 {sreg(S_PF)}, 1")
        I(f"s_cbranch_scc1 {prefix}_STAGED")
    for j in range(NSLOT):
        for op in w_dma(c, j):
            I(op)
        if j < XU:
            for op in x_dma(c, j):
                I(op)
    for r in range(c.nacc):
        I(f"v_accvgpr_write_b32 {areg(r)}, 0")
    I(f"s_waitcnt vmcnt({2 * npw + 8})")
    if persistent:
        I(f"s_branch {prefix}_READY")
        g.L(f"{prefix}_STAGED")
        I(f"s_mov_b32 {sreg(S_WK)}, {128 * NSLOT}")
        I(f"s_min_u32 {sreg(S_WK)}, {sreg(S_WK)}, {sreg(S_WKMAX)}")
        I(f"s_mov_b32 {sreg(S_XK)}, {128 * XU}")
        I(f"s_min_u32 {sreg(S_XK)}, {sreg(S_XK)}, {sreg(S_XKMAX)}")
        for r in range(c.nacc):
            I(f"v_accvgpr_write_b32 {areg(r)}, 0")
        I(f"s_waitcnt vmcnt({n_early})")
        g.L(f"{prefix}_READY")
    I("s_barrier")
    for op in x_frag_reads(c, 0) + w_frag_reads(c, 0):
        I(op)
    I("s_waitcnt lgkmcnt(0)")
    I(f"s_mov_b32 {sreg(S_I)}, 0")
    period = 2 * NSLOT * XU // (2 if NSLOT % 2 == 0 else 1)
    assert (period // 2) % NSLOT == 0 and (period // 2) % XU == 0
    g.L(f"{prefix}_LOOP")
    for h in range(period):
        s = h >> 1
        mm = mfmas(c, h)
        n = len(mm)
        wr = [] if KN("NO_WREAD") else w_frag_reads(c, h + 1)
        if h & 1 == 0:
            fillers = [(0.6 + k * (n - 6) / len(wr), op) for k, op in enumerate(wr)] if wr else []
            xd = x_dma(c, s + 2)
            fillers += spread(drop_loads(xd) if KN("NO_X") else xd, 1.3, n - 1.5)
            g.phase([] if KN("NO_MFMA") else mm, fillers)
            I(f"s_waitcnt vmcnt({npw + 8})")
            I("s_barrier")
        else:
            xr = [] if KN("NO_WREAD") else x_frag_reads(c, s + 1)
            fillers = [(0.3 + k * 0.5, op) for k, op in enumerate(xr)]
            fillers += [(4.6 + k * (n - 10) / len(wr), op) for k, op in enumerate(wr)] if wr else []
            wd = w_dma(c, s + 3)
            fillers += spread(drop_loads(wd) if KN("NO_W") else wd, 1.3, n - 1.5)
            g.phase([] if KN("NO_MFMA") else mm, fillers)
            I(f"s_add_u32 {sreg(S_I)}, {sreg(S_I)}, 1")
            I(f"s_cmp_ge_u32 {sreg(S_I)}, {sreg(S_NK)}")
            I(f"s_cbranch_scc1 {prefix}_EPI")
    I(f"s_branch {prefix}_LOOP")
    g.L(f"{prefix}_EPI")
    I("s_nop 15")
    I("s_nop 15")
    if KN("NO_EPI") and not persistent:
        I("s_waitcnt vmcnt(0)")
        I("s_endpgm")
    if persistent:
        gen_prefetch(g, c, prefix, "A")
    tail_stores = 0 if KN("NO_EPI") else gen_epilogue(g, c)
    if persistent:
        g.L(f"{prefix}_NEXT")
        I(f"s_add_u32 {sreg(S_TILE)}, {sreg(S_TILE)}, {sreg(S_GRID)}")
        I(f"s_cmp_lt_u32 {sreg(S_TILE)}, {sreg(S_NTILES)}")
        I(f"s_cbranch_scc1 {prefix}_TILE")
    I(f"s_waitcnt vmcnt({0 if persistent else min(63, tail_stores)})")
    I("s_endpgm")
    g.L(f"{prefix}_IDLE")
    if persistent:
        I(f"s_cmp_eq_u32 {sreg(S_PF)}, 1")
        I(f"s_cbranch_scc1 {prefix}_IDLE_STAGED")
    for j in range(NSLOT):
        for op in w_dma(c, j):
            I(op)
    I(f"s_waitcnt vmcnt({2 * npw})")
    if persistent:
        I(f"s_branch {prefix}_IDLE_READY")
        g.L(f"{prefix}_IDLE_STAGED")
        I(f"s_mov_b32 {sreg(S_WK)}, {128 * NSLOT}")
        I(f"s_min_u32 {sreg(S_WK)}, {sreg(S_WK)}, {sreg(S_WKMAX)}")
        I("s_waitcnt vmcnt(0)")
        g.L(f"{prefix}_IDLE_READY")
    I("s_barrier")
    I(f"s_mov_b32 {sreg(S_I)}, 0")
    g.L(f"{prefix}_IDLE_LOOP")
    for st in range(NSLOT):
        I(f"s_waitcnt vmcnt({npw})")
        I("s_barrier")
        for op in w_dma(c, st + 3):
            I(op)
        I(f"s_add_u32 {sreg(S_I)}, {sreg(S_I)}, 1")
        I(f"s_cmp_ge_u32 {sreg(S_I)}, {sreg(S_NK)}")
        I(f"s_cbranch_scc1 {prefix}_IDLE_END")
    I(f"s_branch {prefix}_IDLE_LOOP")
    g.L(f"{prefix}_IDLE_END")
    if persistent:
        gen_prefetch(g, c, prefix, "I")
        I(f"s_branch {prefix}_NEXT")
    else:
        I("s_waitcnt vmcnt(0)")
        I("s_endpgm")
    return finalize(g.out)


def gen_prefetch(g: Gen, c: Cfg, prefix: str, tag: str):
    I = g.I
    T = 128
    npw = c.npw
    I("s_barrier")
    I(f"s_mov_b32 {sreg(S_PF)}, 0")
    I(f"s_add_u32 {sreg(S_I)}, {sreg(S_TILE)}, {sreg(S_GRID)}")
    I(f"s_cmp_ge_u32 {sreg(S_I)}, {sreg(S_NTILES)}")
    I(f"s_cbranch_scc1 {prefix}_PF_DONE_{tag}")
    gen_tile_map(g, S_I, T)
    gen_tile_bases(g, c, S_XN, S_WN, S_ROWSN, f"{prefix}_PF_DONE_{tag}", False, prefix)
    I(f"s_mov_b32 {sreg(S_PF)}, 1")
    for rs, base, rows, ld in ((S_WRS, S_WN, None, S_LDW), (S_XRS, S_XN, S_ROWSN, S_LDX)):
        I(f"s_mov_b32 {sreg(rs)}, {sreg(base)}")
        I(f"s_and_b32 {sreg(rs + 1)}, {sreg(base + 1)}, 0xffff")
        if rows is None:
            I(f"s_mul_i32 {sreg(rs + 2)}, {sreg(ld)}, {c.WN}")
        else:
            I(f"s_min_u32 {sreg(S_T0)}, {sreg(rows)}, 256")
            I(f"s_mul_i32 {sreg(rs + 2)}, {sreg(S_T0)}, {sreg(ld)}")
        I(f"s_mov_b32 {sreg(rs + 3)}, 0x00020000")
    I(f"s_mov_b32 {sreg(S_XK)}, 0")
    I(f"s_mov_b32 {sreg(S_WK)}, 0")
    I(f"s_lshl_b32 {sreg(S_T0)}, {sreg(S_WAVE)}, 6")
    I(f"s_cmp_ge_u32 {sreg(S_T0)}, {sreg(S_ROWSN)}")
    I(f"s_cbranch_scc1 {prefix}_PF_WONLY_{tag}")
    for j in range(NSLOT):
        for op in w_dma(c, j):
            I(op)
        if j < XU:
            for op in x_dma(c, j):
                I(op)
    I(f"s_branch {prefix}_PF_DONE_{tag}")
    g.L(f"{prefix}_PF_WONLY_{tag}")
    for j in range(NSLOT):
        for op in w_dma(c, j):
            I(op)
    g.L(f"{prefix}_PF_DONE_{tag}")



def gen_epilogue_setup(g: Gen, c: Cfg):
    I = g.I
    T = c.V_T
    epi = c.epi
    EA = c.V_EA
    for mb in range(c.MB):
        I(f"v_mul_lo_u32 {vreg(EA + mb)}, {vreg(c.V_ROW + mb)}, {sreg(S_LDO)}")
        I(f"v_lshl_add_u32 {vreg(EA + mb)}, {vreg(c.V_H)}, 4, {vreg(EA + mb)}")
    I(f"v_lshlrev_b32 {vreg(EA + 2)}, 3, {vreg(c.V_H)}")
    if epi == EPI_GATE_RES:
        I(f"s_sub_u32 {sreg(S_T1)}, {sreg(S_ROWS)}, 1")
        for mb in range(c.MB):
            m, q, t = T + 66, EA + 3 + mb, T + 48
            I(f"v_min_u32 {vreg(m)}, {sreg(S_T1)}, {vreg(c.V_ROW + mb)}")
            I(f"v_add_u32 {vreg(m)}, {sreg(S_M0)}, {vreg(m)}")
            I(f"v_cvt_f32_u32 {vreg(t)}, {vreg(m)}")
            I(f"v_cvt_f32_u32 {vreg(t + 1)}, {sreg(S_FLEN)}")
            I(f"v_rcp_f32 {vreg(t + 1)}, {vreg(t + 1)}")
            I("s_nop 0")
            I(f"v_mul_f32 {vreg(t)}, {vreg(t)}, {vreg(t + 1)}")
            I(f"v_cvt_u32_f32 {vreg(q)}, {vreg(t)}")
            I(f"v_mul_lo_u32 {vreg(t)}, {vreg(q)}, {sreg(S_FLEN)}")
            I(f"v_cmp_gt_u32_e64 {sreg(S_MSK, 2)}, {vreg(t)}, {vreg(m)}")
            I(f"v_cndmask_b32_e64 {vreg(t + 2)}, 0, 1, {sreg(S_MSK, 2)}")
            I(f"v_sub_u32 {vreg(q)}, {vreg(q)}, {vreg(t + 2)}")
            I(f"v_mul_lo_u32 {vreg(t)}, {vreg(q)}, {sreg(S_FLEN)}")
            I(f"v_add_u32 {vreg(t)}, {sreg(S_FLEN)}, {vreg(t)}")
            I(f"v_cmp_le_u32_e64 {sreg(S_MSK, 2)}, {vreg(t)}, {vreg(m)}")
            I(f"v_cndmask_b32_e64 {vreg(t + 2)}, 0, 1, {sreg(S_MSK, 2)}")
            I(f"v_add_u32 {vreg(q)}, {vreg(q)}, {vreg(t + 2)}")
            I(f"v_mul_lo_u32 {vreg(q)}, {vreg(q)}, {sreg(S_GSTRIDE)}")
            I(f"v_lshl_add_u32 {vreg(q)}, {vreg(c.V_H)}, 3, {vreg(q)}")
    for mb in range(c.MB):
        I(f"v_cmp_lt_u32_e64 {sreg(S_MSK + 2 * mb, 2)}, {vreg(c.V_ROW + mb)}, {sreg(S_ROWS)}")
        I(f"v_cmp_ge_u32_e64 vcc, {vreg(c.V_ROW + mb)}, {sreg(S_ROWLO)}")
        I(f"s_and_b64 {sreg(S_MSK + 2 * mb, 2)}, {sreg(S_MSK + 2 * mb, 2)}, vcc")
    if c.i8:
        I(f"v_lshlrev_b32 {vreg(EA + 5)}, 4, {vreg(c.V_H)}")
        I(f"s_sub_u32 {sreg(S_T1)}, {sreg(S_ROWS)}, 1")
        for mb in range(c.MB):
            I(f"v_min_u32 {vreg(T + 48)}, {sreg(S_T1)}, {vreg(c.V_ROW + mb)}")
            I(f"v_lshlrev_b32 {vreg(T + 48)}, 2, {vreg(T + 48)}")
            I(f"global_load_dword {vreg(c.V_SX + 2 * mb)}, {vreg(T + 48)}, {sreg(S_SX, 2)}")
    n0 = sum(1 for l in g.out if l.startswith("global_load"))
    for nb in range(c.early_nb):
        for g4 in range(4):
            I(f"global_load_dwordx2 {vreg(c.V_EB + 8 * nb + 2 * g4, 2)}, {vreg(EA + 2)}, {sreg(S_BIAS, 2)} offset:{64 * nb + 16 * g4}")
    if c.nl:
        epi_block_loads(g, c, 0, c.V_E0)
    return sum(1 for l in g.out if l.startswith("global_load")) - n0 + (c.MB if c.i8 else 0)


def epi_block_loads(g: Gen, c: Cfg, j: int, P: int):
    I = g.I
    nb, mb = j // c.MB, j % c.MB
    EA = c.V_EA
    if c.epi == EPI_GATE_RES:
        for g4 in range(4):
            I(f"global_load_dwordx2 {vreg(P + 2 * g4, 2)}, {vreg(EA + 3 + mb)}, {sreg(S_GATE, 2)} offset:{64 * nb + 16 * g4}")
    if c.epi in (EPI_GATE_RES, EPI_RES):
        I(f"s_mov_b64 exec, {sreg(S_MSK + 2 * mb, 2)}")
        for k in (0, 2):
            I(f"global_load_dwordx4 {vreg(P + 8 + 2 * k, 4)}, {vreg(EA + mb)}, {sreg(S_RES, 2)} offset:{64 * nb + 16 * k}")
        I("s_mov_b64 exec, -1")


def gen_epilogue(g: Gen, c: Cfg):
    I = g.I
    T = c.V_T
    epi = c.epi
    EA = c.V_EA
    K0, K1, CEXP = 0.7978845608028654, 0.044715, -2.0 * 1.4426950408889634
    cons = {}
    def const_pair(name, val, s0):
        I(f"s_mov_b32 {sreg(s0)}, {hex(f32bits(val))}")
        I(f"s_mov_b32 {sreg(s0 + 1)}, {hex(f32bits(val))}")
        cons[name] = s0
    if epi == EPI_GELU:
        const_pair("k1", K1, 54); const_pair("k0", K0, 56); const_pair("ce", CEXP, 58); const_pair("one", 1.0, 60)
    if epi == EPI_BIAS_SSQ:
        for k in range(2 * c.MB):
            I(f"v_mov_b32 {vreg(c.V_SS + k)}, 0")
    if epi == EPI_PARTIAL:
        for nb in range(c.NB):
            for mb in range(c.MB):
                a0 = c.acc(mb, nb)
                for r in range(16):
                    I(f"v_accvgpr_read_b32 {vreg(T + r)}, {areg(a0 + r)}")
                I(f"s_mov_b64 exec, {sreg(S_MSK + 2 * mb, 2)}")
                for g4 in range(4):
                    I(f"global_store_dwordx4 {vreg(EA + mb)}, {vreg(T + 4 * g4, 4)}, {sreg(S_Y, 2)} offset:{128 * nb + 32 * g4}")
                I("s_mov_b64 exec, -1")
        return 4 * c.NB * c.MB
    BB, PB = T + 72, T + 72 + 8 * c.NB
    assert PB + 32 <= min(c.V_WOFF + 32, 256), (PB, c.V_WOFF)
    n_late = 4 * (c.NB - c.early_nb)
    q = []
    SWB = PB + 32
    assert not c.i8 or SWB + 32 <= c.V_LANE, (SWB, c.V_LANE)

    def wait_for(tags):
        idx = [i for i, t in enumerate(q) if t in tags]
        return None if not idx else min(63, len(q) - 1 - idx[-1])

    def sw_loads(nb):
        for g4 in range(4):
            I(f"global_load_dwordx4 {vreg(SWB + 16 * (nb & 1) + 4 * g4, 4)}, {vreg(EA + 5)}, {sreg(S_SW, 2)} offset:{128 * nb + 32 * g4}")
        q.extend([("sw", nb)] * 4)

    for nb in range(c.early_nb, c.NB):
        for g4 in range(4):
            I(f"global_load_dwordx2 {vreg(BB + 8 * nb + 2 * g4, 2)}, {vreg(EA + 2)}, {sreg(S_BIAS, 2)} offset:{64 * nb + 16 * g4}")
        q.extend([("bias", nb)] * 4)
    if c.i8:
        sw_loads(0)
        for mb in range(c.MB):
            I(f"v_mov_b32 {vreg(c.V_SX + 2 * mb + 1)}, {vreg(c.V_SX + 2 * mb)}")
    blocks = [(nb, mb) for nb in range(c.NB) for mb in range(c.MB)]
    nl = c.nl

    for j, (nb, mb) in enumerate(blocks):
        P = c.V_E0 if j == 0 else PB + 16 * (j & 1)
        if c.i8 and mb == 0 and nb + 1 < c.NB:
            sw_loads(nb + 1)
        if nl and j + 1 < len(blocks):
            epi_block_loads(g, c, j + 1, PB + 16 * ((j + 1) & 1))
            q.extend([("blk", j + 1)] * nl)
        nxt_loads = nl if (nl and j + 1 < len(blocks)) else 0
        if c.i8:
            need = [("blk", j)] + ([("bias", nb), ("sw", nb)] if mb == 0 else [])
            n = wait_for(need)
            if n is not None:
                I(f"s_waitcnt vmcnt({n})")
        elif nl and j == 0:
            I(f"s_waitcnt vmcnt({(n_late if c.early_nb else 0) + nxt_loads})")
        elif nl:
            I(f"s_waitcnt vmcnt({2 + nxt_loads})")
        elif c.early_nb == 0 and j == 0:
            I("s_waitcnt vmcnt(0)")
        if not nl and mb == 0 and nb == c.early_nb and 0 < c.early_nb < c.NB:
            I(f"s_waitcnt vmcnt({min(63, 2 * j)})")
        if mb == 0:
            for g4 in range(4):
                for d in range(2):
                    src = (c.V_EB if nb < c.early_nb else BB) + 8 * nb + 2 * g4 + d
                    I(f"v_lshlrev_b32 {vreg(T + 24 + 4 * g4 + 2 * d)}, 16, {vreg(src)}")
                    I(f"v_and_b32 {vreg(T + 24 + 4 * g4 + 2 * d + 1)}, 0xffff0000, {vreg(src)}")
        a0 = c.acc(mb, nb)
        for r in range(16):
            I(f"v_accvgpr_read_b32 {vreg(T + r)}, {areg(a0 + r)}")
        if c.i8:
            for r in range(16):
                I(f"v_cvt_f32_i32 {vreg(T + r)}, {vreg(T + r)}")
            for r in range(0, 16, 2):
                I(f"v_pk_mul_f32 {vreg(T + 56, 2)}, {vreg(SWB + 16 * (nb & 1) + r, 2)}, {vreg(c.V_SX + 2 * mb, 2)}")
                I(f"v_pk_mul_f32 {vreg(T + r, 2)}, {vreg(T + r, 2)}, {vreg(T + 56, 2)}")
        for r in range(0, 16, 2):
            I(f"v_pk_add_f32 {vreg(T + r, 2)}, {vreg(T + r, 2)}, {vreg(T + 24 + r, 2)}")
        for r in range(0, 16, 2):
            I(f"v_cvt_pk_bf16_f32 {vreg(T + 16 + r // 2)}, {vreg(T + r)}, {vreg(T + r + 1)}")
        if epi in (EPI_GELU, EPI_GATE_RES, EPI_BIAS_SSQ):
            for r in range(0, 16, 2):
                I(f"v_lshlrev_b32 {vreg(T + r)}, 16, {vreg(T + 16 + r // 2)}")
                I(f"v_and_b32 {vreg(T + r + 1)}, 0xffff0000, {vreg(T + 16 + r // 2)}")
        if epi == EPI_BIAS_SSQ:
            for r in range(0, 16, 2):
                I(f"v_pk_fma_f32 {vreg(c.V_SS + 2 * mb, 2)}, {vreg(T + r, 2)}, {vreg(T + r, 2)}, {vreg(c.V_SS + 2 * mb, 2)}")
        if epi == EPI_GATE_RES:
            for r in range(0, 16, 2):
                src = P + r // 2
                I(f"v_lshlrev_b32 {vreg(T + 56)}, 16, {vreg(src)}")
                I(f"v_and_b32 {vreg(T + 57)}, 0xffff0000, {vreg(src)}")
                I(f"v_pk_mul_f32 {vreg(T + r, 2)}, {vreg(T + r, 2)}, {vreg(T + 56, 2)}")
            for r in range(0, 16, 2):
                I(f"v_cvt_pk_bf16_f32 {vreg(T + 16 + r // 2)}, {vreg(T + r)}, {vreg(T + r + 1)}")
        if epi == EPI_GELU:
            for r in range(0, 16, 2):
                x, t = vreg(T + r, 2), vreg(T + 44 + (r % 4), 2)
                I(f"v_pk_mul_f32 {t}, {sreg(cons['k1'], 2)}, {x}")
                I(f"v_pk_mul_f32 {t}, {t}, {x}")
                I(f"v_pk_mul_f32 {t}, {t}, {x}")
                I(f"v_pk_add_f32 {t}, {x}, {t}")
                I(f"v_pk_mul_f32 {t}, {sreg(cons['k0'], 2)}, {t}")
                I(f"v_pk_mul_f32 {t}, {sreg(cons['ce'], 2)}, {t}")
                I(f"v_exp_f32 {vreg(T + 44 + (r % 4))}, {vreg(T + 44 + (r % 4))}")
                I(f"v_exp_f32 {vreg(T + 45 + (r % 4))}, {vreg(T + 45 + (r % 4))}")
                I("s_nop 0")
                I(f"v_pk_add_f32 {t}, {sreg(cons['one'], 2)}, {t}")
                I(f"v_rcp_f32 {vreg(T + 44 + (r % 4))}, {vreg(T + 44 + (r % 4))}")
                I(f"v_rcp_f32 {vreg(T + 45 + (r % 4))}, {vreg(T + 45 + (r % 4))}")
                I("s_nop 0")
                I(f"v_pk_mul_f32 {x}, {x}, {t}")
            for r in range(0, 16, 2):
                I(f"v_cvt_pk_bf16_f32 {vreg(T + 16 + r // 2)}, {vreg(T + r)}, {vreg(T + r + 1)}")
        for k in (0, 2):
            ax, ay, bx, by = T + 16 + 2 * k, T + 17 + 2 * k, T + 18 + 2 * k, T + 19 + 2 * k
            I("s_nop 1")
            I(f"v_permlane32_swap_b32 {vreg(ax)}, {vreg(bx)}")
            I(f"v_permlane32_swap_b32 {vreg(ay)}, {vreg(by)}")
        off_y = 64 * nb
        if epi in (EPI_GATE_RES, EPI_RES):
            for k in (0, 2):
                for d in range(4):
                    vsrc, rsrc = T + 16 + 2 * k + d, P + 8 + 2 * k + d
                    I(f"v_lshlrev_b32 {vreg(T)}, 16, {vreg(vsrc)}")
                    I(f"v_and_b32 {vreg(T + 1)}, 0xffff0000, {vreg(vsrc)}")
                    I(f"v_lshlrev_b32 {vreg(T + 2)}, 16, {vreg(rsrc)}")
                    I(f"v_and_b32 {vreg(T + 3)}, 0xffff0000, {vreg(rsrc)}")
                    I(f"v_pk_add_f32 {vreg(T, 2)}, {vreg(T + 2, 2)}, {vreg(T, 2)}")
                    I(f"v_cvt_pk_bf16_f32 {vreg(vsrc)}, {vreg(T)}, {vreg(T + 1)}")
        I(f"s_mov_b64 exec, {sreg(S_MSK + 2 * mb, 2)}")
        for k in (0, 2):
            I(f"global_store_dwordx4 {vreg(EA + mb)}, {vreg(T + 16 + 2 * k, 4)}, {sreg(S_Y, 2)} offset:{off_y + 16 * k}")
        I("s_mov_b64 exec, -1")
        q.extend([("st", j)] * 2)
    if epi == EPI_BIAS_SSQ:
        for mb in range(c.MB):
            ss = c.V_SS + 2 * mb
            I(f"v_add_f32 {vreg(ss)}, {vreg(ss)}, {vreg(ss + 1)}")
            I(f"v_mov_b32 {vreg(ss + 1)}, {vreg(ss)}")
        I("s_nop 1")
        for mb in range(c.MB):
            ss = c.V_SS + 2 * mb
            I(f"v_permlane32_swap_b32 {vreg(ss)}, {vreg(ss + 1)}")
        for mb in range(c.MB):
            ss = c.V_SS + 2 * mb
            I(f"v_add_f32 {vreg(ss)}, {vreg(ss)}, {vreg(ss + 1)}")
            I(f"v_lshlrev_b32 {vreg(T + mb)}, 2, {vreg(c.V_ROW + mb)}")
            I(f"v_cmp_eq_u32_e64 vcc, {vreg(c.V_H)}, 0")
            I(f"s_and_b64 vcc, vcc, {sreg(S_MSK + 2 * mb, 2)}")
            I("s_mov_b64 exec, vcc")
            I(f"global_store_dword {vreg(T + mb)}, {vreg(ss)}, {sreg(S_SSQ, 2)}")
            I("s_mov_b64 exec, -1")
            q.append(("st", "ssq"))
    n = 0
    while n < len(q) and q[len(q) - 1 - n][0] == "st":
        n += 1
    return n


if __name__ == "__main__":
    if "--diag" in sys.argv:
        sys.argv.remove("--diag")
    WN, epi = int(sys.argv[1]), int(sys.argv[2])
    i8 = len(sys.argv) > 5 and sys.argv[5] == "i8"
    pers = len(sys.argv) > 5 and sys.argv[5] == "p"
    txt = generate(WN, epi, f"GA{WN}E{epi}" + ("I8" if i8 else "") + ("P" if pers else ""), i8, pers)
    probs = lint(txt)
    for p in probs[:20]:
        print("LINT:", p, file=sys.stderr)
    if len(sys.argv) > 3:
        open(sys.argv[3], "w").write(to_inc(txt))
    if len(sys.argv) > 4:
        open(sys.argv[4], "w").write(txt)
    n = sum(1 for l in txt.splitlines() if l and not l.endswith(":"))
    print(f"gemm WN={WN} epi={epi}: {n} instructions, {len(probs)} lint findings", file=sys.stderr)
    sys.exit(1 if probs else 0)
```

### longlive_amd/model.py

```python
from __future__ import annotations

import math
from typing import Dict, List, Optional, Tuple

import torch
import torch.nn as nn

from . import ops
from .kv_cache import KVPlan, plan_update, shadow_refresh_ranges
from .synth import WanConfig

bf16 = torch.bfloat16


class _Lin(nn.Module):
    def __init__(self, out_f: int, in_f: int, device, dtype):
        super().__init__()
        self.weight = nn.Parameter(torch.zeros(out_f, in_f, device=device, dtype=dtype), requires_grad=False)
        self.bias = nn.Parameter(torch.zeros(out_f, device=device, dtype=dtype), requires_grad=False)


class _Norm(nn.Module):
    def __init__(self, dim: int, device, dtype, bias: bool = False):
        super().__init__()
# ... 19 lines not shown
        del self.cross_attn.max_attention_size
        self.norm3 = _Norm(d, device, dtype, bias=True)
        self.ffn = nn.ModuleList([_Lin(cfg.ffn_dim, d, device, dtype), nn.Identity(), _Lin(d, cfg.ffn_dim, device, dtype)])
        self.modulation = nn.Parameter(torch.zeros(1, 6, d, device=device, dtype=dtype), requires_grad=False)


class _Head(nn.Module):
    def __init__(self, cfg: WanConfig, device, dtype):
        super().__init__()
        self.head = _Lin(math.prod(cfg.patch_size) * cfg.out_dim, cfg.dim, device, dtype)
        self.modulation = nn.Parameter(torch.zeros(1, 2, cfg.dim, device=device, dtype=dtype), requires_grad=False)


class _Conv(nn.Module):
    def __init__(self, cfg: WanConfig, device, dtype):
        super().__init__()
        self.weight = nn.Parameter(torch.zeros(cfg.dim, cfg.in_dim, *cfg.patch_size, device=device, dtype=dtype),
                                   requires_grad=False)
        self.bias = nn.Parameter(torch.zeros(cfg.dim, device=device, dtype=dtype), requires_grad=False)


_MX_SHADOW = "_ll_mx"


def mx_shadow_key(k: torch.Tensor, v: torch.Tensor) -> tuple:
    return (k.data_ptr(), v.data_ptr(), tuple(k.shape), k._version, v._version)


def _idx_versions(cache: dict):
    g, e = cache.get("global_end_index"), cache.get("local_end_index")
    return (g._version if torch.is_tensor(g) else ("int", g), e._version if torch.is_tensor(e) else ("int", e))


def _kv_state(cache: dict) -> Tuple[int, int]:
    st = cache.get("_ll_idx")
    if st is not None and len(st) == 4 and st[2:] != list(_idx_versions(cache)):
        st = None
    if st is None:
        g, e = cache["global_end_index"], cache["local_end_index"]
        st = [int(g.item()) if torch.is_tensor(g) else int(g), int(e.item()) if torch.is_tensor(e) else int(e),
              *_idx_versions(cache)]
        cache["_ll_idx"] = st
    return st[0], st[1]


def _kv_commit(cache: dict, G: int, E: int) -> None:
    for key, val in (("global_end_index", G), ("local_end_index", E)):
        cur = cache.get(key)
        if torch.is_tensor(cur):
            cur.fill_(val)
        else:
            cache[key] = val
    cache["_ll_idx"] = [G, E, *_idx_versions(cache)]


class CausalWanModelHIP(nn.Module):

    def __init__(self, cfg: WanConfig, device="cuda", dtype=bf16):
        super().__init__()
        assert dtype == bf16, "the HIP path computes in bf16 (inference.py:134)"
        assert cfg.head_dim == 128, "kernels are specialised for head_dim 128 (Wan2.1-T2V-1.3B: 1536 / 12)"
        assert cfg.patch_size == (1, 2, 2)
        self.cfg = cfg
        d = cfg.dim
        self.patch_embedding = _Conv(cfg, device, dtype)
        self.text_embedding = nn.ModuleList([_Lin(d, cfg.text_dim, device, dtype), nn.Identity(), _Lin(d, d, device, dtype)])
        self.time_embedding = nn.ModuleList([_Lin(d, cfg.freq_dim, device, dtype), nn.Identity(), _Lin(d, d, device, dtype)])
        self.time_projection = nn.ModuleList([nn.Identity(), _Lin(6 * d, d, device, dtype)])
        self.blocks = nn.ModuleList([_Block(cfg, device, dtype) for _ in range(cfg.num_layers)])
        self.head = _Head(cfg, device, dtype)
        self.local_attn_size = cfg.local_attn_size
        self.sink_size = cfg.sink_size
        self.max_attention_size = 32760 if cfg.local_attn_size == -1 else cfg.local_attn_size * 1560
        for b in self.blocks:
            b.self_attn.max_attention_size = self.max_attention_size
        self.num_frame_per_block = 1
        self.block_mask = None
        self.quant: Optional[str] = None
        self.attn_quant: Optional[str] = None
        self.use_modulation_table = True
        self.fuse_v_insert = True
        self.use_modulation_f32 = True
        self.fuse_cross_qnorm = True
        self._packed = None
        self._rope_f = None
        self._rope_hw: Dict[Tuple[int, int], torch.Tensor] = {}
        self._ctx_cache = None
        self._time_memo: Dict[tuple, tuple] = {}
        self._register_load_state_dict_pre_hook(self._invalidate_derived)

    def _apply(self, fn, *a, **k):
        self._packed = None
        self._rope_f = None
        self._rope_hw = {}
        self._ctx_cache = None
        self._time_memo = {}
        return super()._apply(fn, *a, **k)

    def _invalidate_derived(self, *unused_hook_args):
        self._packed = None
        self._ctx_cache = None
        self._time_memo = {}

    def invalidate_packed(self):
        self._invalidate_derived()

    def load_state_dict(self, state_dict, strict: bool = True, **kw):
        self._invalidate_derived()
        return super().load_state_dict(state_dict, strict=strict, **kw)

    @staticmethod
    def _prepare_blockwise_causal_attn_mask(*args, **kwargs):
        return None

    def _param_key(self):
        key = []
        for blk in self.blocks:
            sa = blk.self_attn
            ts = [sa.q.weight, sa.k.weight, sa.v.weight, sa.q.bias, sa.k.bias, sa.v.bias, blk.modulation]
            if self.quant in ("int8", "mxfp8", "fp8_rowwise", "mxfp6", "mxfp4_a6", "mxfp4_a4"):
                ts += [sa.o.weight, blk.cross_attn.q.weight, blk.cross_attn.o.weight, blk.ffn[0].weight, blk.ffn[2].weight]
            key.extend((t.data_ptr(), t._version) for t in ts)
        return tuple(key)

    def _pack(self):
        if self._packed is not None:
            if self._packed_key == self._param_key():
                return self._packed
            self._invalidate_derived()
        P = []
        for blk in self.blocks:
            sa, ca = blk.self_attn, blk.cross_attn
            d = dict(
                wqkv=torch.cat([sa.q.weight, sa.k.weight, sa.v.weight], 0).contiguous(),
                bqkv=torch.cat([sa.q.bias, sa.k.bias, sa.v.bias], 0).contiguous(),
                mod=blk.modulation.detach().reshape(6, -1).contiguous(),
            )
            if self.quant is not None:
                quantize = {"int8": ops.quantize_rows, "mxfp8": ops.quantize_mx, "fp8_rowwise": ops.quantize_rows_f8,
                            "mxfp6": ops.quantize_mx6, "mxfp4_a6": ops.quantize_mx4, "mxfp4_a4": ops.quantize_mx4}[self.quant]
                for name, w in (("qkv", d["wqkv"]), ("o", sa.o.weight), ("cq", ca.q.weight), ("co", ca.o.weight),
                                ("f1", blk.ffn[0].weight), ("f2", blk.ffn[2].weight)):
                    d["q_" + name], d["s_" + name] = quantize(w.detach().contiguous())
            P.append(d)
        self._packed = P
        self._mods = torch.stack([d["mod"] for d in P], 0).contiguous()
        self._packed_key = self._param_key()
        return P

    def set_quant(self, mode: Optional[str]):
        if mode not in (None, "int8", "mxfp8", "fp8_rowwise", "mxfp6", "mxfp4_a6", "mxfp4_a4"):
            raise ValueError(f"unknown quantisation mode {mode!r}")
        if mode is not None and (self.cfg.dim % 128 or self.cfg.ffn_dim % 128):
            raise ValueError(f"{mode} linears need dim and ffn_dim to be multiples of 128")
        if mode in ("mxfp6", "mxfp4_a6", "mxfp4_a4") and (self.cfg.dim % 256 or self.cfg.ffn_dim % 256):
            raise ValueError(f"{mode} linears need dim and ffn_dim to be multiples of 256 (packed 256-k super-blocks)")
        self.quant = mode
        self._packed = None
        return self

    def set_attn_quant(self, mode: Optional[str]):
        if mode not in (None, "mxfp8"):
            raise ValueError(f"unknown attention quantisation mode {mode!r}")
        if mode is not None and self.cfg.head_dim != 128:
            raise ValueError("MX attention needs head_dim 128")
        self.attn_quant = mode
        return self

    @staticmethod
    def _mx_shadow(kvc: dict):
        k = kvc["k"]
        sh = kvc.get(_MX_SHADOW)
        if sh is None or sh["kq"].shape[0] != k.shape[0] or sh["S"] != k.shape[1] or sh["kq"].shape[2] != k.shape[2]:
            sh = ops.kv_shadow_mx_alloc(k)
            sh["key"] = None
            kvc[_MX_SHADOW] = sh
        return sh, sh["key"] != mx_shadow_key(k, kvc["v"])

    def _lin(self, x, pk, key, w, b, epilogue=0, **kw):
        if self.quant == "mxfp4_a4":
            xm = x if isinstance(x, tuple) else ops.quantize_mx4(x)
            return ops.gemm_mx4(xm, (pk["q_" + key], pk["s_" + key]), b, epilogue, tag="gemm_" + key, **kw)
        if self.quant == "mxfp4_a6":
            xm = x if isinstance(x, tuple) else ops.quantize_mx6(x)
            return ops.gemm_mx4w6(xm, (pk["q_" + key], pk["s_" + key]), b, epilogue, tag="gemm_" + key, **kw)
        if self.quant == "mxfp6":
            xm = x if isinstance(x, tuple) else ops.quantize_mx6(x)
            return ops.gemm_mx6(xm, (pk["q_" + key], pk["s_" + key]), b, epilogue, tag="gemm_" + key, **kw)
        if self.quant == "fp8_rowwise":
            xq, sx = x if isinstance(x, tuple) else ops.quantize_rows_f8(x)
            return ops.gemm_f8(xq, sx, pk["q_" + key], pk["s_" + key], b, epilogue, tag="gemm_" + key, **kw)
        if self.quant == "mxfp8":
            xm = x if isinstance(x, tuple) else ops.quantize_mx(x)
            return ops.gemm_mx(xm, (pk["q_" + key], pk["s_" + key]), b, epilogue, tag="gemm_" + key, **kw)
        if self.quant == "int8":
            xq, sx = x if isinstance(x, tuple) else ops.quantize_rows(x)
            return ops.gemm_w8a8(xq, sx, pk["q_" + key], pk["s_" + key], b, epilogue, tag="gemm_" + key, **kw)
        return ops.gemm(x, w, b, epilogue, tag="gemm_" + key, **kw)

    def _rope_tables(self, hp: int, wp: int, device):
        d = self.cfg.head_dim
        half = d // 2
        c3 = half // 3
        nf = half - 2 * c3

        def angles(n, dim):
            return torch.outer(torch.arange(n, dtype=torch.float64),
                               1.0 / torch.pow(10000.0, torch.arange(0, dim, 2, dtype=torch.float64).div(dim)))

        if self._rope_f is None:
            a = angles(1024, d - 4 * (d // 6))
            assert a.shape[1] == nf
            self._rope_f = torch.stack([a.cos(), a.sin()], -1).float().contiguous().to(device)
        key = (hp, wp)
        if key not in self._rope_hw:
            ah = angles(1024, 2 * (d // 6))[:hp]
            aw = angles(1024, 2 * (d // 6))[:wp]
            a = torch.cat([ah.view(hp, 1, c3).expand(hp, wp, c3), aw.view(1, wp, c3).expand(hp, wp, c3)], -1)
            a = a.reshape(hp * wp, 2 * c3)
            self._rope_hw[key] = torch.stack([a.cos(), a.sin()], -1).float().contiguous().to(device)
        return self._rope_f, self._rope_hw[key]

    def time_embed(self, t: torch.Tensor):
        c = self.cfg
        tf = t.reshape(-1).to(torch.float32).contiguous()
        emb = ops.sinusoid(tf, c.freq_dim)
        h = ops.linear_small(emb, self.time_embedding[0].weight, self.time_embedding[0].bias, act_out=1)
        e = ops.linear_small(h, self.time_embedding[2].weight, self.time_embedding[2].bias)
        e0 = ops.linear_small(e, self.time_projection[1].weight, self.time_projection[1].bias, act_in=1)
        return e, e0.view(*t.shape, 6, c.dim)

# ... 26 lines not shown
        B, L, C = xs.shape
        Hh, D = c.num_heads, c.head_dim
        hp, wp = grid_hw
        fs = hp * wp
        if L != F * fs:
            raise ValueError(f"block_forward: {L} tokens are not {F} frames of {hp}x{wp}")
        rope_f, rope_hw = self._rope_tables(hp, wp, xs.device)
        if q_buf is None:
            q_buf = torch.empty(B, L, Hh, D, dtype=bf16, device=xs.device)
        blk = self.blocks[i]
        if pk is None:
            pk = self._pack()[i]
        mod = None if premod else pk["mod"]
        sa, ca = blk.self_attn, blk.cross_attn
        q8 = self.quant == "int8"
        mx = self.quant == "mxfp8"
        f8 = self.quant == "fp8_rowwise"
        m6 = self.quant in ("mxfp6", "mxfp4_a6")
        m4 = self.quant == "mxfp4_a4"
        G, E = _kv_state(kvc)
        S = kvc["k"].shape[1]
        plan = plan_update(current_start, L, G, E, S, self.sink_size * fs, self.local_attn_size,
                           sa.max_attention_size, sink_recache_after_switch)
        amx = self.attn_quant == "mxfp8"
        if amx:
            shadow, stale = self._mx_shadow(kvc)
        else:
            kvc.pop(_MX_SHADOW, None)
        if plan.roll is not None:
            ops.kv_roll(kvc["k"], kvc["v"], *plan.roll)
        if mx:
            h1 = ops.ln_modulate_tab_mx(xs, tab32, 0, 1, F, c.eps) if tab32 is not None else ops.ln_modulate_mx(xs, e0, mod, 0, 1, F, c.eps)
        elif m6:
            h1 = ops.ln_modulate_tab_mx6(xs, tab32, 0, 1, F, c.eps) if tab32 is not None else ops.ln_modulate_mx6(xs, e0, mod, 0, 1, F, c.eps)
        elif m4:
            h1 = ops.ln_modulate_tab_mx4(xs, tab32, 0, 1, F, c.eps) if tab32 is not None else ops.ln_modulate_mx4(xs, e0, mod, 0, 1, F, c.eps)
        elif f8:
            h1 = ops.ln_modulate_tab_f8(xs, tab32, 0, 1, F, c.eps) if tab32 is not None else ops.ln_modulate_f8(xs, e0, mod, 0, 1, F, c.eps)
        elif tab32 is not None:
            h1 = ops.ln_modulate_tab(xs, tab32, 0, 1, F, c.eps, q8=q8)
        else:
            h1 = (ops.ln_modulate_q8 if q8 else ops.ln_modulate)(xs, e0, mod, 0, 1, F, c.eps)
        if self.fuse_v_insert:
            if mx:
                qkv = ops.gemm_mx_qkv_v_insert(h1, (pk["q_qkv"], pk["s_qkv"]), pk["bqkv"], kvc["v"], plan.write_start,
                                               plan.roped_offset, plan.write_len, B, L)
            elif m6:
                qkv_m6 = ops.gemm_mx4w6_qkv_v_insert if self.quant == "mxfp4_a6" else ops.gemm_mx6_qkv_v_insert
                qkv = qkv_m6(h1, (pk["q_qkv"], pk["s_qkv"]), pk["bqkv"], kvc["v"], plan.write_start, plan.roped_offset, plan.write_len,
                             B, L)
            elif m4:
                qkv = ops.gemm_mx4_qkv_v_insert(h1, (pk["q_qkv"], pk["s_qkv"]), pk["bqkv"], kvc["v"], plan.write_start,
                                                plan.roped_offset, plan.write_len, B, L)
            elif f8:
                qkv = ops.gemm_f8_qkv_v_insert(h1, (pk["q_qkv"], pk["s_qkv"]), pk["bqkv"], kvc["v"], plan.write_start,
                                               plan.roped_offset, plan.write_len, B, L)
            elif q8:
                qkv = ops.gemm_qkv_v_insert(None, (pk["q_qkv"], pk["s_qkv"]), pk["bqkv"], kvc["v"], plan.write_start,
                                            plan.roped_offset, plan.write_len, xq=h1)
            else:
                qkv = ops.gemm_qkv_v_insert(h1, pk["wqkv"], pk["bqkv"], kvc["v"], plan.write_start, plan.roped_offset,
                                            plan.write_len)
            v_dst = None
        else:
            qkv = self._lin(h1, pk, "qkv", pk["wqkv"], pk["bqkv"])
            v_dst = kvc["v"]
        ops.qk_norm_rope_kv_store(qkv, sa.norm_q.weight, sa.norm_k.weight, rope_f, rope_hw, q_buf.view(B, L, C),
                                  kvc["k"], v_dst, D, fs, current_start // fs, plan.write_start,
                                  plan.roped_offset, plan.write_len, c.eps)
        if amx:
            for lo, hi in shadow_refresh_ranges(plan, stale, S):
                ops.kv_shadow_mx(kvc["k"], kvc["v"], shadow, lo, hi, tag="kv_shadow_mx_co" if co_running else "kv_shadow_mx")
            shadow["key"] = mx_shadow_key(kvc["k"], kvc["v"])
        if kv_insert_only:
            if cache_done_event is not None:
                cache_done_event.record(torch.cuda.current_stream())
            return plan
        if amx:
            att = ops.flash_attn_mx(q_buf, shadow, plan.segments, tag="flash_attn_self_mx_co" if co_running else "flash_attn_self_mx")
        else:
            att = ops.flash_attn(q_buf, kvc["k"], kvc["v"], plan.segments, tag="flash_attn_self_co" if co_running else "flash_attn_self")
        if cache_done_event is not None:
            cache_done_event.record(torch.cuda.current_stream())
        self._lin(att.view(B, L, C), pk, "o", sa.o.weight, sa.o.bias, ops.EPI_BIAS_GATE_RES, out=xs, res=xs, e=e0,
                  mod=mod, gate_idx=2, rows_per_batch=L, frame_len=fs)
        xn = (ops.layernorm_affine_mx if mx else ops.layernorm_affine_mx6 if m6 else ops.layernorm_affine_mx4 if m4 else ops.layernorm_affine_f8 if f8 else ops.layernorm_affine_q8 if q8 else
              ops.layernorm_affine)(xs, blk.norm3.weight, blk.norm3.bias, c.eps)
        fuse_qn = (self.fuse_cross_qnorm and self.quant is None and ops.gemm_ssq_planes(B * L, C, C) == Hh and ops.flash_attn_qnorm_ok(Hh, c.text_len))
        if fuse_qn:
            qraw, ssq = ops.gemm_ssq(xn, ca.q.weight, ca.q.bias, tag="gemm_cq_ssq")
        else:
            qc = ops.rmsnorm(self._lin(xn, pk, "cq", ca.q.weight, ca.q.bias), ca.norm_q.weight, c.eps)
        if not cac["is_init"]:
            kc = ops.gemm(ctx, ca.k.weight, ca.k.bias)
            if cac["k"].shape != (B, c.text_len, Hh, D) or not cac["k"].is_contiguous():
                cac["k"] = torch.empty(B, c.text_len, Hh, D, dtype=bf16, device=xs.device)
                cac["v"] = torch.empty(B, c.text_len, Hh, D, dtype=bf16, device=xs.device)
            ops.rmsnorm(kc, ca.norm_k.weight, c.eps, out=cac["k"].view(B, c.text_len, C))
            ops.gemm(ctx, ca.v.weight, ca.v.bias, out=cac["v"].view(B, c.text_len, C))
            cac["is_init"] = True
        if fuse_qn:
            atc = ops.flash_attn_qnorm(qraw.view(B, L, Hh, D), ssq, ca.norm_q.weight, c.eps, cac["k"], cac["v"], c.text_len, tag="flash_attn_cross_qn")
        else:
            atc = ops.flash_attn(qc.view(B, L, Hh, D), cac["k"], cac["v"], [(0, c.text_len)], tag="flash_attn_cross")
        self._lin(atc.view(B, L, C), pk, "co", ca.o.weight, ca.o.bias, ops.EPI_BIAS_RES, out=xs, res=xs)
        if mx:
            h2 = ops.ln_modulate_tab_mx(xs, tab32, 3, 4, F, c.eps) if tab32 is not None else ops.ln_modulate_mx(xs, e0, mod, 3, 4, F, c.eps)
        elif m6:
            h2 = ops.ln_modulate_tab_mx6(xs, tab32, 3, 4, F, c.eps) if tab32 is not None else ops.ln_modulate_mx6(xs, e0, mod, 3, 4, F, c.eps)
        elif m4:
            h2 = ops.ln_modulate_tab_mx4(xs, tab32, 3, 4, F, c.eps) if tab32 is not None else ops.ln_modulate_mx4(xs, e0, mod, 3, 4, F, c.eps)
        elif f8:
            h2 = ops.ln_modulate_tab_f8(xs, tab32, 3, 4, F, c.eps) if tab32 is not None else ops.ln_modulate_f8(xs, e0, mod, 3, 4, F, c.eps)
        elif tab32 is not None:
            h2 = ops.ln_modulate_tab(xs, tab32, 3, 4, F, c.eps, q8=q8)
        else:
            h2 = (ops.ln_modulate_q8 if q8 else ops.ln_modulate)(xs, e0, mod, 3, 4, F, c.eps)
        ff = self._lin(h2, pk, "f1", blk.ffn[0].weight, blk.ffn[0].bias, ops.EPI_BIAS_GELU,
                       **(dict(mx_out=True) if mx or m6 or m4 else {}))
        self._lin(ff, pk, "f2", blk.ffn[2].weight, blk.ffn[2].bias, ops.EPI_BIAS_GATE_RES, out=xs, res=xs, e=e0,
                  mod=mod, gate_idx=5, rows_per_batch=L, frame_len=fs)
        return plan

    @torch.no_grad()
    def forward_frames(self, x: torch.Tensor, t: torch.Tensor, context: torch.Tensor, kv_cache: List[dict],
                       crossattn_cache: List[dict], current_start: int = 0,
                       sink_recache_after_switch: bool = False, sigma: Optional[torch.Tensor] = None,
                       kv_only: bool = False, layer_wait=None, layer_record=None, t_uniform: Optional[float] = None):
        c = self.cfg
        B, F, Cin, H, W = x.shape
        hp, wp = H // 2, W // 2
        fs = hp * wp
        L = F * fs
        Hh, D, C = c.num_heads, c.head_dim, c.dim
        assert current_start % fs == 0, "current_start must sit on a frame boundary"
        x = x.to(bf16).contiguous()
        pe = self.patch_embedding
        xs = ops.gemm(ops.patchify(x), pe.weight.view(C, -1), pe.bias)
        need_ctx = any(not cc["is_init"] for cc in crossattn_cache)
        ctx = self.text_embed(context) if need_ctx else None

        q_buf = torch.empty(B, L, Hh, D, dtype=bf16, device=x.device)
        plans: List[KVPlan] = []
        last = len(self.blocks) - 1
        P = self._pack()
        premod = self.use_modulation_table
        tab_f32 = premod and self.use_modulation_f32 and x.is_cuda
        memo_key = None
        if t_uniform is not None and x.is_cuda and tuple(t.shape) == (B, F):
            memo_key = (float(t_uniform), B, F, premod, tab_f32, torch.cuda.current_stream(x.device).cuda_stream)
            hit = self._time_memo.get(memo_key)
            if hit is not None and hit[0] == self._time_param_key() and hit[1] is self._packed_key:
                e, e0, etab, etab32 = hit[2:]
            else:
                hit = None
        if memo_key is None or hit is None:
            e, e0 = self.time_embed(t)
            etab = ops.modulation_table(e0, self._mods) if premod else None
            etab32 = ops.modulation_table_f32(e0, self._mods, 0b010010) if tab_f32 else None
            if memo_key is not None:
                if len(self._time_memo) >= 64:
                    self._time_memo = {}
                self._time_memo[memo_key] = (self._time_param_key(), self._packed_key, e, e0, etab, etab32)
        cur_stream = torch.cuda.current_stream() if (layer_wait is not None or layer_record is not None) else None
        for i in range(len(self.blocks)):
            if layer_wait is not None:
                cur_stream.wait_event(layer_wait[i])
            plans.append(self.block_forward(i, xs, etab[i] if premod else e0, ctx, kv_cache[i], crossattn_cache[i], F, (hp, wp),
                                            current_start, sink_recache_after_switch, q_buf,
                                            kv_insert_only=kv_only and i == last, pk=P[i], premod=premod,
                                            cache_done_event=layer_record[i] if layer_record is not None else None,
                                            co_running=cur_stream is not None, tab32=etab32[i] if tab_f32 else None))
# ... 23 lines not shown
```

### longlive_amd/ops.py

```python
from __future__ import annotations

import math
from typing import Optional, Tuple

import torch

from . import _lib

bf16 = torch.bfloat16

EPI_BIAS, EPI_BIAS_GELU, EPI_BIAS_GATE_RES, EPI_BIAS_RES = 0, 1, 2, 3


def _stream() -> int:
    return torch.cuda.current_stream().cuda_stream


class KernelTimer:

    def __init__(self, tags=None):
        self.tags = None if tags is None else set(tags)
        self.records = {}
        self.base = torch.cuda.Event(enable_timing=True)
        self.base.record()
# ... 205 lines not shown
    assert rope_f.shape == (1024, nf, 2), rope_f.shape
    assert rope_hw.shape == (frame_len, half - nf, 2), rope_hw.shape
    lib = _lib.load()
    t0 = _t0("qk_norm_rope_kv_store")
    _lib.check(lib.ll_qk_norm_rope_kv_store(qkv.data_ptr(), wq.data_ptr(), wk.data_ptr(), rope_f.data_ptr(),
                                            rope_hw.data_ptr(), q_out.data_ptr(), cache_k.data_ptr(),
                                            _ptr(cache_v), B, L, Cc, head_dim, frame_len, start_frame, S,
                                            write_start, roped_offset, write_len, eps, _stream()),
               "ll_qk_norm_rope_kv_store")
    nv = 1 if cache_v is not None else 0
    _t1("qk_norm_rope_kv_store", t0, 2.0 * ((2 + nv) * B * L * Cc + B * L * Cc + (1 + nv) * B * write_len * Cc))
    return q_out


def kv_roll(cache_k, cache_v, dst: int, src: int, n: int):
    _chk(cache_k, "cache_k"); _chk(cache_v, "cache_v")
    B, S = cache_k.shape[:2]
    Cc = cache_k.numel() // (B * S)
    assert cache_v.shape == cache_k.shape
    lib = _lib.load()
    t0 = _t0("kv_roll")
    _lib.check(lib.ll_kv_roll(cache_k.data_ptr(), cache_v.data_ptr(), B, S, Cc, dst, src, n, _stream()), "ll_kv_roll")
    _t1("kv_roll", t0, 2.0 * 2 * 2 * B * n * Cc)


def gemm(x, w, bias, epilogue: int = EPI_BIAS, out=None, res=None, e=None, mod=None, gate_idx: int = 0,
         rows_per_batch: int = 0, frame_len: int = 0, tag: str = "gemm"):
    _chk(x, "x"); _chk(w, "w"); _chk(bias, "bias")
    K = x.shape[-1]
    M = x.numel() // K
    N = w.shape[0]
    assert w.shape == (N, K) and bias.numel() == N, (w.shape, bias.shape, K)
    if out is None:
        out = torch.empty(*x.shape[:-1], N, dtype=bf16, device=x.device)
    _chk(out, "out")
    assert out.numel() == M * N
    nmod = 0
    if epilogue in (EPI_BIAS_GATE_RES, EPI_BIAS_RES):
        _chk(res, "res")
        assert res.numel() == M * N
    if epilogue == EPI_BIAS_GATE_RES:
        _chk(e, "e")
        nmod = e.shape[-2]
        assert e.shape[-1] == N and e.numel() == (M // frame_len) * nmod * N, (e.shape, M, frame_len)
        if mod is not None:
            _chk(mod, "mod")
            assert mod.numel() == nmod * N
    lib = _lib.load()
    t0 = _t0(tag)
    if M <= 1024 and M * N <= (1 << 22) and epilogue in (EPI_BIAS, EPI_BIAS_RES) and _ksplit_plan(lib, M, N, K):
        ws = ksplit_workspace(x.device, M, N, K)
        _lib.check(lib.ll_gemm_bf16_ksplit(x.data_ptr(), w.data_ptr(), bias.data_ptr(), out.data_ptr(), M, N, K, K, N, epilogue,
                                           _ptr(res), ws.data_ptr(), ws.numel(), _stream()), "ll_gemm_bf16_ksplit")
    else:
        _lib.check(lib.ll_gemm_bf16(x.data_ptr(), w.data_ptr(), bias.data_ptr(), out.data_ptr(), M, N, K, K, N, epilogue,
                                    _ptr(res), _ptr(e), _ptr(mod), nmod, gate_idx, rows_per_batch, frame_len, _stream()),
                   "ll_gemm_bf16")
    _t1(tag, t0, 2.0 * M * N * K)
    return out


def gemm_ssq_planes(M: int, N: int, K: int) -> int:
    return int(_lib.load().ll_gemm_ssq_planes(M, N, K))


def gemm_ssq(x, w, bias, out=None, tag: str = "gemm"):
    _chk(x, "x"); _chk(w, "w"); _chk(bias, "bias")
    K = x.shape[-1]
    M = x.numel() // K
    N = w.shape[0]
    assert w.shape == (N, K) and bias.numel() == N
    if out is None:
        out = torch.empty(*x.shape[:-1], N, dtype=bf16, device=x.device)
    _chk(out, "out")
    assert out.numel() == M * N
    planes = gemm_ssq_planes(M, N, K)
    if planes == 0:
        raise RuntimeError(f"gemm_ssq: {M} x {N} x {K} is not covered by the generated kernel (use gemm + rmsnorm)")
    ssq = torch.empty(planes, M, dtype=torch.float32, device=x.device)
    lib = _lib.load()
    t0 = _t0(tag)
    _lib.check(lib.ll_gemm_bf16_ssq(x.data_ptr(), w.data_ptr(), bias.data_ptr(), out.data_ptr(), ssq.data_ptr(), M, N, K, K, N, _stream()),
               "ll_gemm_bf16_ssq")
    _t1(tag, t0, 2.0 * M * N * K)
    return out, ssq


_ksplit_ws = {}


def _ksplit_plan(lib, M: int, N: int, K: int) -> int:
    return int(lib.ll_gemm_ksplit_plan(M, N, K))


def _dev_index(device) -> int:
    return torch.cuda.current_device() if device.index is None else device.index


def ksplit_workspace(device, M: int, N: int, K: int) -> torch.Tensor:
    need = int(_lib.load().ll_gemm_ksplit_workspace_bytes(M, N, K))
    key = (device.type, _dev_index(device), int(_stream() or 0))
    buf = _ksplit_ws.get(key)
    if buf is None or buf.numel() < need:
        buf = torch.empty(max(need, 16), dtype=torch.uint8, device=device)
        _ksplit_ws[key] = buf
    return buf


def gemm_qkv_v_insert(x, w, bias, cache_v, write_start: int, roped_offset: int, write_len: int, xq=None, tag: str = "gemm_qkv"):
    _chk(bias, "bias"); _chk(cache_v, "cache_v")
    int8 = xq is not None
    if int8:
        xi, sx = xq
        wq, sw = w
        _chk(xi, "xq", torch.int8); _chk(sx, "sx", torch.float32); _chk(wq, "wq", torch.int8); _chk(sw, "sw", torch.float32)
        B, L, K = xi.shape
        N = wq.shape[0]
        assert wq.shape == (N, K) and sx.numel() == B * L and sw.numel() == N
        dev = xi.device
    else:
        _chk(x, "x"); _chk(w, "w")
        B, L, K = x.shape
        N = w.shape[0]
        assert w.shape == (N, K)
        dev = x.device
    assert bias.numel() == N and N % 3 == 0
    S = cache_v.shape[1]
    assert cache_v.shape[0] == B and cache_v.numel() == B * S * (N // 3), (cache_v.shape, B, S, N)
    out = torch.empty(B, L, N, dtype=bf16, device=dev)
    lib = _lib.load()
    t0 = _t0(tag)
    if int8:
        _lib.check(lib.ll_gemm_w8a8_qkv(xi.data_ptr(), sx.data_ptr(), wq.data_ptr(), sw.data_ptr(), bias.data_ptr(), out.data_ptr(),
                                        B * L, N, K, N, cache_v.data_ptr(), B, L, S, write_start, roped_offset, write_len, _stream()),
                   "ll_gemm_w8a8_qkv")
    else:
        _lib.check(lib.ll_gemm_bf16_qkv(x.data_ptr(), w.data_ptr(), bias.data_ptr(), out.data_ptr(), B * L, N, K, K, N,
                                        cache_v.data_ptr(), B, L, S, write_start, roped_offset, write_len, _stream()),
                   "ll_gemm_bf16_qkv")
    _t1(tag, t0, 2.0 * B * L * N * K)
    return out


def quantize_rows(x, q=None, scale=None):
    _chk(x, "x")
    K = x.shape[-1]
    rows = x.numel() // K
    if q is None:
        q = torch.empty(x.shape, dtype=torch.int8, device=x.device)
    if scale is None:
        scale = torch.empty(rows, dtype=torch.float32, device=x.device)
    _chk(q, "q", torch.int8); _chk(scale, "scale", torch.float32)
    assert q.numel() == x.numel() and scale.numel() == rows
    lib = _lib.load()
    t0 = _t0("quantize_rows")
    _lib.check(lib.ll_quantize_rows(x.data_ptr(), q.data_ptr(), scale.data_ptr(), rows, K, K, _stream()), "ll_quantize_rows")
    _t1("quantize_rows", t0, 3.0 * x.numel())
    return q, scale


def gemm_w8a8(xq, sx, wq, sw, bias, epilogue: int = EPI_BIAS, out=None, res=None, e=None, mod=None, gate_idx: int = 0,
              rows_per_batch: int = 0, frame_len: int = 0, tag: str = "gemm"):
    _chk(xq, "xq", torch.int8); _chk(wq, "wq", torch.int8); _chk(sx, "sx", torch.float32); _chk(sw, "sw", torch.float32)
    _chk(bias, "bias")
    K = xq.shape[-1]
    M = xq.numel() // K
# ... 979 lines not shown
```

Before: 91.62.

## Fold norm3 layernorm into cross-attn q GEMM via o-proj row stats

The self-attention output GEMM (gate+residual epilogue) now also emits per-row partial sum and sum-of-squares planes. The cross-attention q GEMM consumes the raw residual stream with a weight premultiplied by the norm3 affine scale, then reconstructs the layernorm algebraically from those stats plus cached per-column s and c vectors. This removes the standalone layernorm_affine pass and its normalized activation tensor. In exchange it adds two generated assembly kernel variants, a cached weight-premod step, and possible numerical drift from folding the normalization after the matmul.

```diff
diff --git a/include/longlive_hip.h b/include/longlive_hip.h
--- a/include/longlive_hip.h
+++ b/include/longlive_hip.h
@@ -174,6 +174,16 @@
 int ll_gemm_bf16_ssq(const ll_bf16* x, const ll_bf16* w, const ll_bf16* bias, ll_bf16* out, float* ssq, int M, int N, int K, int ldx,
                      int ldo, ll_stream stream);
 int ll_flash_attn_qnorm_ok(int H, int nkeys);
+
+int ll_lnfold_premod(const ll_bf16* w, const float* a, const float* t, const ll_bf16* bias, ll_bf16* wp, float* svec, float* cvec,
+                     int N, int K, ll_stream stream);
+int ll_gemm_stats_planes(int M, int N, int K, int frame_len);
+int ll_gemm_bf16_gate_res_stats(const ll_bf16* x, const ll_bf16* w, const ll_bf16* bias, ll_bf16* out, float* stats, int M, int N, int K,
+                                int ldx, int ldo, const ll_bf16* res, const ll_bf16* e, int nmod, int gate_idx, int rows_per_batch,
+                                int frame_len, ll_stream stream);
+int ll_gemm_lnfold_ssq_planes(int M, int N, int K);
+int ll_gemm_lnfold_ssq(const ll_bf16* x, const ll_bf16* wp, const float* svec, const float* cvec, const float* stats, float eps,
+                       ll_bf16* out, float* ssq, int M, int N, int K, int ldo, ll_stream stream);
 int ll_flash_attn_qnorm(const ll_bf16* q, const float* ssq, const ll_bf16* norm_w, float eps, const ll_bf16* k, const ll_bf16* v,
                         ll_bf16* out, int B, int Lq, int H, int ldq, int ldo, int ldk, long long k_batch_stride, int key_start,
                         int nkeys, float scale, ll_stream stream);
diff --git a/longlive_amd/_lib.py b/longlive_amd/_lib.py
--- a/longlive_amd/_lib.py
+++ b/longlive_amd/_lib.py
@@ -47,6 +47,11 @@
     "ll_gemm_ssq_planes": [_i, _i, _i],
     "ll_gemm_bf16_ssq": [_p, _p, _p, _p, _p, _i, _i, _i, _i, _i, _p],
     "ll_flash_attn_qnorm_ok": [_i, _i],
+    "ll_lnfold_premod": [_p] * 7 + [_i, _i, _p],
+    "ll_gemm_stats_planes": [_i, _i, _i, _i],
+    "ll_gemm_bf16_gate_res_stats": [_p] * 5 + [_i] * 5 + [_p, _p] + [_i] * 4 + [_p],
+    "ll_gemm_lnfold_ssq_planes": [_i, _i, _i],
+    "ll_gemm_lnfold_ssq": [_p] * 5 + [_f, _p, _p] + [_i] * 4 + [_p],
     "ll_flash_attn_qnorm": [_p, _p, _p, _f, _p, _p, _p, _i, _i, _i, _i, _i, _i, _ll, _i, _i, _f, _p],
     "ll_conv_cl": [_p] * 6 + [_i] * 10 + [_p],
     "ll_conv_cl_rms_ok": [_i] * 7,
diff --git a/longlive_amd/csrc/elementwise.hip b/longlive_amd/csrc/elementwise.hip
--- a/longlive_amd/csrc/elementwise.hip
+++ b/longlive_amd/csrc/elementwise.hip
@@ -972,6 +972,44 @@
   return ll_check_launch("ll_modulation_table_f32");
 }
 
+__global__ __launch_bounds__(256) void lnfold_premod_kernel(const bf16* __restrict__ w, const float* __restrict__ a,
+                                                            const float* __restrict__ t, const bf16* __restrict__ bias,
+                                                            bf16* __restrict__ wp, float* __restrict__ svec, float* __restrict__ cvec, int K) {
+  __shared__ double sh[2][256];
+  const int n = blockIdx.x;
+  double ss = 0.0, cc = 0.0;
+  for (int k = threadIdx.x; k < K; k += 256) {
+    const float wv = (float)w[(size_t)n * K + k];
+    const bf16 p = (bf16)(wv * a[k]);
+    wp[(size_t)n * K + k] = p;
+    ss += (double)(float)p;
+    cc += (double)t[k] * (double)wv;
+  }
+  sh[0][threadIdx.x] = ss;
+  sh[1][threadIdx.x] = cc;
+  __syncthreads();
+  for (int d = 128; d > 0; d >>= 1) {
+    if ((int)threadIdx.x < d) {
+      sh[0][threadIdx.x] += sh[0][threadIdx.x + d];
+      sh[1][threadIdx.x] += sh[1][threadIdx.x + d];
+    }
+    __syncthreads();
+  }
+  if (threadIdx.x == 0) {
+    svec[n] = (float)sh[0][0];
+    cvec[n] = (float)(sh[1][0] + (double)(float)bias[n]);
+  }
+}
+
+extern "C" int ll_lnfold_premod(const ll_bf16* w, const float* a, const float* t, const ll_bf16* bias, ll_bf16* wp, float* svec,
+                                float* cvec, int N, int K, ll_stream stream) {
+  LL_REQUIRE(w && a && t && bias && wp && svec && cvec, "ll_lnfold_premod: every operand is required");
+  LL_REQUIRE(N > 0 && K > 0, "ll_lnfold_premod: bad shape %d x %d", N, K);
+  hipLaunchKernelGGL(lnfold_premod_kernel, dim3((unsigned)N), dim3(256), 0, (hipStream_t)stream, (const bf16*)w, a, t, (const bf16*)bias,
+                     (bf16*)wp, svec, cvec, K);
+  return ll_check_launch("ll_lnfold_premod");
+}
+
 extern "C" int ll_ln_modulate_tab(const ll_bf16* x, ll_bf16* out, int8_t* q, float* qscale, const float* tab, int nmod,
                                   int shift_idx, int scale_idx, int B, int L, int C, int F, float eps, ll_stream stream) {
   LL_REQUIRE(row_ok(C), "ll_ln_modulate_tab: C=%d must be a multiple of 8 and <= 2048", C);
diff --git a/longlive_amd/csrc/gemm.hip b/longlive_amd/csrc/gemm.hip
--- a/longlive_amd/csrc/gemm.hip
+++ b/longlive_amd/csrc/gemm.hip
@@ -596,6 +596,52 @@
   return ll_check_launch("ll_gemm_bf16_ssq");
 }
 
+bool gemm_asm_stats_ok(int M, int N, int K, int frame_len);
+int gemm_asm_stats_launch(const bf16* x, const bf16* w, bf16* out, float* stats, int M, int N, int K, int ldx, int ldo, const EpiArgs& ea,
+                          int gm, hipStream_t s);
+bool gemm_asm_lnfold_ssq_ok(int M, int N, int K);
+int gemm_asm_lnfold_ssq_launch(const bf16* x, const bf16* w, const float* svec, const float* cvec, const float* stats, float eps, bf16* out,
+                               float* ssq, int M, int N, int K, int ldo, int gm, hipStream_t s);
+extern "C" int ll_gemm_stats_planes(int M, int N, int K, int frame_len) {
+  if (!gemm_asm_wanted(LL_EPI_BIAS_GATE_RES)) return 0;
+  return gemm_asm_stats_ok(M, N, K, frame_len) ? N / 128 : 0;
+}
+extern "C" int ll_gemm_bf16_gate_res_stats(const ll_bf16* x, const ll_bf16* w, const ll_bf16* bias, ll_bf16* out, float* stats, int M, int N,
+                                           int K, int ldx, int ldo, const ll_bf16* res, const ll_bf16* e, int nmod, int gate_idx,
+                                           int rows_per_batch, int frame_len, ll_stream stream) {
+  LL_REQUIRE(K > 0 && K % 64 == 0, "ll_gemm_bf16_gate_res_stats: K=%d must be a positive multiple of 64", K);
+  int rc = check_epilogue("ll_gemm_bf16_gate_res_stats", M, N, ldo, LL_EPI_BIAS_GATE_RES, bias, res, e, nullptr, nmod, gate_idx, rows_per_batch,
+                          frame_len);
+  if (rc) return rc;
+  LL_REQUIRE(stats != nullptr && ((size_t)stats & 3) == 0, "ll_gemm_bf16_gate_res_stats: stats is required");
+  LL_REQUIRE(ll_gemm_stats_planes(M, N, K, frame_len) > 0 && ldx == K, "ll_gemm_bf16_gate_res_stats: %d x %d x %d is not covered by the generated "
+             "kernel under the current tuning (ask ll_gemm_stats_planes first and run ll_gemm_bf16 instead)", M, N, K);
+  EpiArgs ea{(const bf16*)bias, (const bf16*)res, (const bf16*)e, nullptr, nullptr, nullptr, nmod, gate_idx,
+             rows_per_batch, frame_len, rows_per_batch / frame_len};
+  const int r = gemm_asm_stats_launch((const bf16*)x, (const bf16*)w, (bf16*)out, stats, M, N, K, ldx, ldo, ea, g_gemm_group_m, (hipStream_t)stream);
+  if (r < 0) return r;
+  LL_REQUIRE(r == 1, "ll_gemm_bf16_gate_res_stats: the generated kernel refused a shape its plan accepted");
+  return ll_check_launch("ll_gemm_bf16_gate_res_stats");
+}
+extern "C" int ll_gemm_lnfold_ssq_planes(int M, int N, int K) {
+  if (!gemm_asm_wanted(LL_EPI_BIAS)) return 0;
+  return gemm_asm_lnfold_ssq_ok(M, N, K) && N / 128 <= 16 ? N / 128 : 0;
+}
+extern "C" int ll_gemm_lnfold_ssq(const ll_bf16* x, const ll_bf16* wp, const float* svec, const float* cvec, const float* stats, float eps,
+                                  ll_bf16* out, float* ssq, int M, int N, int K, int ldo, ll_stream stream) {
+  LL_REQUIRE(x && wp && svec && cvec && stats && out && ssq, "ll_gemm_lnfold_ssq: every operand is required");
+  LL_REQUIRE(((size_t)svec & 15) == 0 && ((size_t)cvec & 15) == 0 && ((size_t)stats & 3) == 0 && ((size_t)ssq & 3) == 0,
+             "ll_gemm_lnfold_ssq: s and c must be 16-byte aligned, stats and ssq 4-byte aligned");
+  LL_REQUIRE(N > 0 && ldo >= N && ldo % 4 == 0, "ll_gemm_lnfold_ssq: ldo=%d must be >= N=%d and a multiple of 4", ldo, N);
+  LL_REQUIRE(M > 0 && ll_gemm_lnfold_ssq_planes(M, N, K) > 0, "ll_gemm_lnfold_ssq: %d x %d x %d is not covered by the generated kernel under the "
+             "current tuning (ask ll_gemm_lnfold_ssq_planes first and run ll_layernorm_affine + ll_gemm_bf16_ssq instead)", M, N, K);
+  const int r = gemm_asm_lnfold_ssq_launch((const bf16*)x, (const bf16*)wp, svec, cvec, stats, eps, (bf16*)out, ssq, M, N, K, ldo, g_gemm_group_m,
+                                           (hipStream_t)stream);
+  if (r < 0) return r;
+  LL_REQUIRE(r == 1, "ll_gemm_lnfold_ssq: the generated kernel refused a shape its plan accepted");
+  return ll_check_launch("ll_gemm_lnfold_ssq");
+}
+
 extern "C" int ll_gemm_ksplit_plan(int M, int N, int K) {
   if (!gemm_asm_wanted(LL_EPI_BIAS)) return 0;
   return gemm_ksplit_splits(M, N, K, device_cus());
diff --git a/longlive_amd/csrc/gemm_asm.hip b/longlive_amd/csrc/gemm_asm.hip
--- a/longlive_amd/csrc/gemm_asm.hip
+++ b/longlive_amd/csrc/gemm_asm.hip
@@ -74,6 +74,27 @@
 #define GA_INC "build/gemm_asm_128_5.inc"
 #define GA_SSQ 1
 #include "gemm_asm_kernel.inl"
+#undef GA_SSQ
+#undef GA_NAME
+#undef GA_WN
+#undef GA_INC
+
+#define GA_NAME gemm_asm_128_gate_res_stats
+#define GA_WN 128
+#define GA_INC "build/gemm_asm_128_6.inc"
+#define GA_STATS 1
+#include "gemm_asm_kernel.inl"
+#undef GA_STATS
+#undef GA_NAME
+#undef GA_WN
+#undef GA_INC
+#define GA_NAME gemm_asm_128_lnfold_ssq
+#define GA_WN 128
+#define GA_INC "build/gemm_asm_128_7.inc"
+#define GA_SSQ 1
+#define GA_LNFOLD 1
+#include "gemm_asm_kernel.inl"
+#undef GA_LNFOLD
 #undef GA_SSQ
 #undef GA_NAME
 #undef GA_WN
@@ -212,6 +233,49 @@
   return 1;
 }
 
+bool gemm_asm_stats_ok(int M, int N, int K, int frame_len) {
+  if (gemm_asm_width(M, N, K, K, LL_EPI_BIAS_GATE_RES, true, false, false, frame_len) != 128) return false;
+  return (long long)2 * (N / 128) * M * 4 < 0x7fffffffLL;
+}
+int gemm_asm_stats_launch(const bf16* x, const bf16* w, bf16* out, float* stats, int M, int N, int K, int ldx, int ldo, const EpiArgs& ea,
+                          int gm, hipStream_t s) {
+  if (ldx != K || !gemm_asm_stats_ok(M, N, K, ea.frame_len) || ea.sx != nullptr || ea.mod != nullptr || ea.v_out != nullptr) return 0;
+  const void* fn = (const void*)gemm_asm_128_gate_res_stats;
+  const int lds = 3 * 128 * 128 + 4 * 2 * 8192;
+  if (int rc = ll_lds_attr(fn, lds)) return rc;
+  const int ntm = (M + 255) / 256, ntn = N / 128;
+  const bf16* gate = ea.e + (size_t)ea.gate_idx * N;
+  const int gstride = ea.nmod * N * 2;
+  bf16* nov = nullptr;
+  int zero = 0;
+  void* args[] = {(void*)&x, (void*)&w, (void*)&ea.bias, (void*)&out, (void*)&ea.res, (void*)&gate, (void*)&M, (void*)&N, (void*)&K,
+                  (void*)&ldx, (void*)&ldo, (void*)&ea.frame_len, (void*)&gstride, (void*)&ntm, (void*)&ntn, (void*)&gm,
+                  (void*)&nov, (void*)&zero, (void*)&zero, (void*)&zero, (void*)&zero, (void*)&zero, (void*)&stats};
+  if (hipLaunchKernel(fn, dim3(ntm * ntn), dim3(256), args, (size_t)lds, s) != hipSuccess) return ll_check_launch("gemm_asm_128_gate_res_stats");
+  return 1;
+}
+
+bool gemm_asm_lnfold_ssq_ok(int M, int N, int K) {
+  return K == 1536 && gemm_asm_width(M, N, K, K, LL_EPI_BIAS, true, false, false, 0) == 128 && (long long)24 * M * 4 < 0x7fffffffLL;
+}
+int gemm_asm_lnfold_ssq_launch(const bf16* x, const bf16* w, const float* svec, const float* cvec, const float* stats, float eps, bf16* out,
+                               float* ssq, int M, int N, int K, int ldo, int gm, hipStream_t s) {
+  if (!gemm_asm_lnfold_ssq_ok(M, N, K)) return 0;
+  const void* fn = (const void*)gemm_asm_128_lnfold_ssq;
+  const int lds = 3 * 128 * 128 + 4 * 2 * 8192;
+  if (int rc = ll_lds_attr(fn, lds)) return rc;
+  const int ntm = (M + 255) / 256, ntn = N / 128;
+  const bf16* nullb = nullptr;
+  bf16* nov = nullptr;
+  int zero = 0, ldx = K;
+  void* args[] = {(void*)&x, (void*)&w, (void*)&nullb, (void*)&out, (void*)&nullb, (void*)&nullb, (void*)&M, (void*)&N, (void*)&K,
+                  (void*)&ldx, (void*)&ldo, (void*)&zero, (void*)&zero, (void*)&ntm, (void*)&ntn, (void*)&gm,
+                  (void*)&nov, (void*)&zero, (void*)&zero, (void*)&zero, (void*)&zero, (void*)&zero, (void*)&ssq, (void*)&stats,
+                  (void*)&svec, (void*)&cvec, (void*)&eps};
+  if (hipLaunchKernel(fn, dim3(ntm * ntn), dim3(256), args, (size_t)lds, s) != hipSuccess) return ll_check_launch("gemm_asm_128_lnfold_ssq");
+  return 1;
+}
+
 const char* gemm_asm_plan(int M, int N, int wn, int epilogue, char* out, int cap, bool i8) {
   const char* tail = wn == 224 ? "gelu" : wn == 256 ? "bias" : epilogue == LL_EPI_BIAS ? "bias" : epilogue == LL_EPI_BIAS_GATE_RES ? "gate_res" : "res";
   const int tiles = ((M + 255) / 256) * (N / wn), cus = gemm_asm_cus() & ~7;
diff --git a/longlive_amd/csrc/gen/gemm_asm_gen.py b/longlive_amd/csrc/gen/gemm_asm_gen.py
--- a/longlive_amd/csrc/gen/gemm_asm_gen.py
+++ b/longlive_amd/csrc/gen/gemm_asm_gen.py
@@ -11,6 +11,9 @@
 EPI_BIAS, EPI_GELU, EPI_GATE_RES, EPI_RES = 0, 1, 2, 3
 EPI_PARTIAL = 4
 EPI_BIAS_SSQ = 5
+EPI_GATE_RES_STATS = 6
+EPI_LNFOLD_SSQ = 7
+LNFOLD_PLANES = 12
 
 S_X, S_W, S_Y, S_BIAS, S_RES, S_GATE = 8, 10, 12, 14, 16, 18
 S_LDX, S_LDW, S_LDO = 20, 21, 22
@@ -19,6 +22,8 @@
 S_ROWLO = 29
 S_SX, S_SW = 64, 66
 S_SSQ = 64
+S_STAT, S_STATP2 = 64, 66
+S_LNSTAT, S_LNPS, S_LNEPS, S_LNS = 66, 68, 69, 70
 S_XRS, S_WRS = 32, 36
 S_WAVE, S_I, S_T0, S_T1, S_T2 = 40, 41, 44, 45, 46
 S_WM0, S_XK, S_WK, S_XKMAX, S_WKMAX = 47, 48, 49, 43, 62
@@ -43,7 +48,10 @@
 class Cfg:
     def __init__(self, WN, epi, i8=False):
         assert WN % 32 == 0 and 64 <= WN <= 256
-        assert not (i8 and epi in (EPI_PARTIAL, EPI_BIAS_SSQ))
+        self.stats, self.lnfold = epi == EPI_GATE_RES_STATS, epi == EPI_LNFOLD_SSQ
+        epi = EPI_GATE_RES if self.stats else EPI_BIAS_SSQ if self.lnfold else epi
+        assert not (i8 and (epi in (EPI_PARTIAL, EPI_BIAS_SSQ) or self.stats))
+        assert WN == 128 or not (self.stats or self.lnfold)
         self.WN, self.NB, self.MB, self.epi, self.i8 = WN, WN // 32, 2, epi, i8
         self.nacc = self.MB * self.NB * 16
         self.slotb = WN * 128
@@ -72,9 +80,14 @@
         self.V_E0 = top
         top += 16 if self.nl else 0
         self.V_SS = top
-        top += 4 if epi == EPI_BIAS_SSQ else 0
+        top += 4 if epi == EPI_BIAS_SSQ and not self.lnfold else 0
+        self.V_ST = top
+        top += 8 if self.stats else 0
         self.V_EB = top
         self.early_nb = 0 if epi == EPI_PARTIAL else max(0, min(self.NB, (256 - top) // 8))
+        if self.lnfold:
+            self.V_MR, self.V_SC, self.V_SS, self.early_nb = top, top + 4, self.V_T + 64, 0
+            assert self.V_SC + 64 <= 256, self.V_SC
 
     def acc(self, mb, nb):
         return (mb * self.NB + nb) * 16
@@ -252,7 +265,7 @@
 
 def generate(WN: int, epi: int, prefix: str, i8: bool = False, persistent: bool = False) -> str:
     c = Cfg(WN, epi, i8)
-    assert not (persistent and (i8 or epi in (EPI_PARTIAL, EPI_BIAS_SSQ)))
+    assert not (persistent and (i8 or c.epi in (EPI_PARTIAL, EPI_BIAS_SSQ) or c.stats))
     g = Gen()
     I = g.I
     T = 128
@@ -330,6 +343,8 @@
     for r in range(c.nacc):
         I(f"v_accvgpr_write_b32 {areg(r)}, 0")
     I(f"s_waitcnt vmcnt({2 * npw + 8})")
+    if c.lnfold:
+        gen_lnfold_rowstats(g, c)
     if persistent:
         I(f"s_branch {prefix}_READY")
         g.L(f"{prefix}_STAGED")
@@ -474,7 +489,7 @@
     for mb in range(c.MB):
         I(f"v_mul_lo_u32 {vreg(EA + mb)}, {vreg(c.V_ROW + mb)}, {sreg(S_LDO)}")
         I(f"v_lshl_add_u32 {vreg(EA + mb)}, {vreg(c.V_H)}, 4, {vreg(EA + mb)}")
-    I(f"v_lshlrev_b32 {vreg(EA + 2)}, 3, {vreg(c.V_H)}")
+    I(f"v_lshlrev_b32 {vreg(EA + 2)}, {4 if c.lnfold else 3}, {vreg(c.V_H)}")
     if epi == EPI_GATE_RES:
         I(f"s_sub_u32 {sreg(S_T1)}, {sreg(S_ROWS)}, 1")
         for mb in range(c.MB):
@@ -510,12 +525,53 @@
             I(f"v_lshlrev_b32 {vreg(T + 48)}, 2, {vreg(T + 48)}")
             I(f"global_load_dword {vreg(c.V_SX + 2 * mb)}, {vreg(T + 48)}, {sreg(S_SX, 2)}")
     n0 = sum(1 for l in g.out if l.startswith("global_load"))
+    if c.lnfold:
+        I(f"s_sub_u32 {sreg(S_T1)}, {sreg(S_ROWS)}, 1")
+        for mb in range(c.MB):
+            I(f"v_min_u32 {vreg(T + 48 + mb)}, {sreg(S_T1)}, {vreg(c.V_ROW + mb)}")
+            I(f"v_lshlrev_b32 {vreg(T + 48 + mb)}, 2, {vreg(T + 48 + mb)}")
+        for p in range(2 * LNFOLD_PLANES):
+            for mb in range(c.MB):
+                I(f"global_load_dword {vreg(T + 2 * p + mb)}, {vreg(T + 48 + mb)}, {sreg(S_LNSTAT, 2)}")
+                if p + 1 < 2 * LNFOLD_PLANES:
+                    I(f"v_add_u32 {vreg(T + 48 + mb)}, {sreg(S_LNPS)}, {vreg(T + 48 + mb)}")
+        for nb in range(2):
+            lnfold_sc_loads(g, c, nb)
     for nb in range(c.early_nb):
         for g4 in range(4):
             I(f"global_load_dwordx2 {vreg(c.V_EB + 8 * nb + 2 * g4, 2)}, {vreg(EA + 2)}, {sreg(S_BIAS, 2)} offset:{64 * nb + 16 * g4}")
     if c.nl:
         epi_block_loads(g, c, 0, c.V_E0)
     return sum(1 for l in g.out if l.startswith("global_load")) - n0 + (c.MB if c.i8 else 0)
+
+
+def lnfold_sc_loads(g: Gen, c: Cfg, nb: int):
+    B = c.V_SC + 32 * (nb & 1)
+    for base, sr in ((B, S_LNS), (B + 16, S_BIAS)):
+        for g4 in range(4):
+            g.I(f"global_load_dwordx4 {vreg(base + 4 * g4, 4)}, {vreg(c.V_EA + 2)}, {sreg(sr, 2)} offset:{128 * nb + 32 * g4}")
+    return 8
+
+
+def gen_lnfold_rowstats(g: Gen, c: Cfg):
+    I = g.I
+    T, NP = c.V_T, LNFOLD_PLANES
+    for kind in range(2):
+        a = T + 2 * NP * kind
+        for p in range(1, NP):
+            I(f"v_pk_add_f32 {vreg(a, 2)}, {vreg(a, 2)}, {vreg(a + 2 * p, 2)}")
+    inv = hex(f32bits(1.0 / (128 * NP)))
+    for mb in range(c.MB):
+        su, sq, t = T + mb, T + 2 * NP + mb, T + 50 + mb
+        I(f"v_mul_f32 {vreg(su)}, {inv}, {vreg(su)}")
+        I(f"v_mul_f32 {vreg(sq)}, {inv}, {vreg(sq)}")
+        I(f"v_mul_f32 {vreg(t)}, {vreg(su)}, {vreg(su)}")
+        I(f"v_sub_f32 {vreg(sq)}, {vreg(sq)}, {vreg(t)}")
+        I(f"v_max_f32 {vreg(sq)}, 0, {vreg(sq)}")
+        I(f"v_add_f32 {vreg(sq)}, {sreg(S_LNEPS)}, {vreg(sq)}")
+        I(f"v_rsq_f32 {vreg(c.V_MR + 2 + mb)}, {vreg(sq)}")
+        I(f"v_sub_f32 {vreg(c.V_MR + mb)}, 0, {vreg(su)}")
+    I("s_nop 0")
 
 
 def epi_block_loads(g: Gen, c: Cfg, j: int, P: int):
@@ -548,6 +604,9 @@
     if epi == EPI_BIAS_SSQ:
         for k in range(2 * c.MB):
             I(f"v_mov_b32 {vreg(c.V_SS + k)}, 0")
+    if c.stats:
+        for k in range(4 * c.MB):
+            I(f"v_mov_b32 {vreg(c.V_ST + k)}, 0")
     if epi == EPI_PARTIAL:
         for nb in range(c.NB):
             for mb in range(c.MB):
@@ -575,7 +634,7 @@
             I(f"global_load_dwordx4 {vreg(SWB + 16 * (nb & 1) + 4 * g4, 4)}, {vreg(EA + 5)}, {sreg(S_SW, 2)} offset:{128 * nb + 32 * g4}")
         q.extend([("sw", nb)] * 4)
 
-    for nb in range(c.early_nb, c.NB):
+    for nb in range(c.NB if c.lnfold else c.early_nb, c.NB):
         for g4 in range(4):
             I(f"global_load_dwordx2 {vreg(BB + 8 * nb + 2 * g4, 2)}, {vreg(EA + 2)}, {sreg(S_BIAS, 2)} offset:{64 * nb + 16 * g4}")
         q.extend([("bias", nb)] * 4)
@@ -603,11 +662,15 @@
             I(f"s_waitcnt vmcnt({(n_late if c.early_nb else 0) + nxt_loads})")
         elif nl:
             I(f"s_waitcnt vmcnt({2 + nxt_loads})")
+        elif c.lnfold:
+            n = wait_for([("sc", nb)]) if mb == 0 else None
+            if n is not None:
+                I(f"s_waitcnt vmcnt({n})")
         elif c.early_nb == 0 and j == 0:
             I("s_waitcnt vmcnt(0)")
         if not nl and mb == 0 and nb == c.early_nb and 0 < c.early_nb < c.NB:
             I(f"s_waitcnt vmcnt({min(63, 2 * j)})")
-        if mb == 0:
+        if mb == 0 and not c.lnfold:
             for g4 in range(4):
                 for d in range(2):
                     src = (c.V_EB if nb < c.early_nb else BB) + 8 * nb + 2 * g4 + d
@@ -622,7 +685,18 @@
             for r in range(0, 16, 2):
                 I(f"v_pk_mul_f32 {vreg(T + 56, 2)}, {vreg(SWB + 16 * (nb & 1) + r, 2)}, {vreg(c.V_SX + 2 * mb, 2)}")
                 I(f"v_pk_mul_f32 {vreg(T + r, 2)}, {vreg(T + r, 2)}, {vreg(T + 56, 2)}")
-        for r in range(0, 16, 2):
+        if c.lnfold:
+            SB = c.V_SC + 32 * (nb & 1)
+            for k in range(2):
+                I(f"v_mov_b32 {vreg(T + 40 + k)}, {vreg(c.V_MR + mb)}")
+                I(f"v_mov_b32 {vreg(T + 42 + k)}, {vreg(c.V_MR + 2 + mb)}")
+            for r in range(0, 16, 2):
+                I(f"v_pk_fma_f32 {vreg(T + r, 2)}, {vreg(T + 40, 2)}, {vreg(SB + r, 2)}, {vreg(T + r, 2)}")
+            for r in range(0, 16, 2):
+                I(f"v_pk_fma_f32 {vreg(T + r, 2)}, {vreg(T + 42, 2)}, {vreg(T + r, 2)}, {vreg(SB + 16 + r, 2)}")
+            if mb == c.MB - 1 and nb + 2 < c.NB:
+                q.extend([("sc", nb + 2)] * lnfold_sc_loads(g, c, nb + 2))
+        for r in range(0, 16, 2) if not c.lnfold else ():
             I(f"v_pk_add_f32 {vreg(T + r, 2)}, {vreg(T + r, 2)}, {vreg(T + 24 + r, 2)}")
         for r in range(0, 16, 2):
             I(f"v_cvt_pk_bf16_f32 {vreg(T + 16 + r // 2)}, {vreg(T + r)}, {vreg(T + r + 1)}")
@@ -676,28 +750,37 @@
                     I(f"v_and_b32 {vreg(T + 3)}, 0xffff0000, {vreg(rsrc)}")
                     I(f"v_pk_add_f32 {vreg(T, 2)}, {vreg(T + 2, 2)}, {vreg(T, 2)}")
                     I(f"v_cvt_pk_bf16_f32 {vreg(vsrc)}, {vreg(T)}, {vreg(T + 1)}")
+                    if c.stats:
+                        I(f"v_lshlrev_b32 {vreg(T + 4)}, 16, {vreg(vsrc)}")
+                        I(f"v_and_b32 {vreg(T + 5)}, 0xffff0000, {vreg(vsrc)}")
+                        I(f"v_pk_add_f32 {vreg(c.V_ST + 4 * mb, 2)}, {vreg(c.V_ST + 4 * mb, 2)}, {vreg(T + 4, 2)}")
+                        I(f"v_pk_fma_f32 {vreg(c.V_ST + 4 * mb + 2, 2)}, {vreg(T + 4, 2)}, {vreg(T + 4, 2)}, {vreg(c.V_ST + 4 * mb + 2, 2)}")
         I(f"s_mov_b64 exec, {sreg(S_MSK + 2 * mb, 2)}")
         for k in (0, 2):
             I(f"global_store_dwordx4 {vreg(EA + mb)}, {vreg(T + 16 + 2 * k, 4)}, {sreg(S_Y, 2)} offset:{off_y + 16 * k}")
         I("s_mov_b64 exec, -1")
         q.extend([("st", j)] * 2)
+    sums = []
     if epi == EPI_BIAS_SSQ:
-        for mb in range(c.MB):
-            ss = c.V_SS + 2 * mb
+        sums = [(c.V_SS + 2 * mb, mb, S_SSQ, None) for mb in range(c.MB)]
+    if c.stats:
+        sums = [(c.V_ST + 4 * mb + 2 * k, mb, S_STAT, S_STATP2 if k else None) for mb in range(c.MB) for k in range(2)]
+    if sums:
+        for ss, mb, base, poff in sums:
             I(f"v_add_f32 {vreg(ss)}, {vreg(ss)}, {vreg(ss + 1)}")
             I(f"v_mov_b32 {vreg(ss + 1)}, {vreg(ss)}")
         I("s_nop 1")
-        for mb in range(c.MB):
-            ss = c.V_SS + 2 * mb
+        for ss, mb, base, poff in sums:
             I(f"v_permlane32_swap_b32 {vreg(ss)}, {vreg(ss + 1)}")
-        for mb in range(c.MB):
-            ss = c.V_SS + 2 * mb
+        for i, (ss, mb, base, poff) in enumerate(sums):
             I(f"v_add_f32 {vreg(ss)}, {vreg(ss)}, {vreg(ss + 1)}")
-            I(f"v_lshlrev_b32 {vreg(T + mb)}, 2, {vreg(c.V_ROW + mb)}")
+            I(f"v_lshlrev_b32 {vreg(T + i)}, 2, {vreg(c.V_ROW + mb)}")
+            if poff is not None:
+                I(f"v_add_u32 {vreg(T + i)}, {sreg(poff)}, {vreg(T + i)}")
             I(f"v_cmp_eq_u32_e64 vcc, {vreg(c.V_H)}, 0")
             I(f"s_and_b64 vcc, vcc, {sreg(S_MSK + 2 * mb, 2)}")
             I("s_mov_b64 exec, vcc")
-            I(f"global_store_dword {vreg(T + mb)}, {vreg(ss)}, {sreg(S_SSQ, 2)}")
+            I(f"global_store_dword {vreg(T + i)}, {vreg(ss)}, {sreg(base, 2)}")
             I("s_mov_b64 exec, -1")
             q.append(("st", "ssq"))
     n = 0
diff --git a/longlive_amd/model.py b/longlive_amd/model.py
--- a/longlive_amd/model.py
+++ b/longlive_amd/model.py
@@ -125,6 +125,8 @@
         self.fuse_v_insert = True
         self.use_modulation_f32 = True
         self.fuse_cross_qnorm = True
+        self.fold_layernorm = True
+        self._lnfold: Dict[int, tuple] = {}
         self._packed = None
         self._rope_f = None
         self._rope_hw: Dict[Tuple[int, int], torch.Tensor] = {}
@@ -138,12 +140,14 @@
         self._rope_hw = {}
         self._ctx_cache = None
         self._time_memo = {}
+        self._lnfold = {}
         return super()._apply(fn, *a, **k)
 
     def _invalidate_derived(self, *unused_hook_args):
         self._packed = None
         self._ctx_cache = None
         self._time_memo = {}
+        self._lnfold = {}
 
     def invalidate_packed(self):
         self._invalidate_derived()
@@ -190,6 +194,21 @@
         self._mods = torch.stack([d["mod"] for d in P], 0).contiguous()
         self._packed_key = self._param_key()
         return P
+
+    @staticmethod
+    def lnfold_key(*params) -> tuple:
+        return tuple((p.data_ptr(), p._version) for p in params)
+
+    def _lnfold_norm3(self, i: int):
+        blk = self.blocks[i]
+        ps = (blk.cross_attn.q.weight, blk.cross_attn.q.bias, blk.norm3.weight, blk.norm3.bias)
+        key = self.lnfold_key(*ps)
+        hit = self._lnfold.get(i)
+        if hit is None or hit[0] != key:
+            hit = (key, ops.lnfold_premod(ps[0].detach(), ps[2].detach().float().contiguous(), ps[3].detach().float().contiguous(),
+                                          ps[1].detach()))
+            self._lnfold[i] = hit
+        return hit[1]
 
     def set_quant(self, mode: Optional[str]):
         if mode not in (None, "int8", "mxfp8", "fp8_rowwise", "mxfp6", "mxfp4_a6", "mxfp4_a4"):
@@ -382,12 +401,19 @@
             att = ops.flash_attn(q_buf, kvc["k"], kvc["v"], plan.segments, tag="flash_attn_self_co" if co_running else "flash_attn_self")
         if cache_done_event is not None:
             cache_done_event.record(torch.cuda.current_stream())
-        self._lin(att.view(B, L, C), pk, "o", sa.o.weight, sa.o.bias, ops.EPI_BIAS_GATE_RES, out=xs, res=xs, e=e0,
-                  mod=mod, gate_idx=2, rows_per_batch=L, frame_len=fs)
-        xn = (ops.layernorm_affine_mx if mx else ops.layernorm_affine_mx6 if m6 else ops.layernorm_affine_mx4 if m4 else ops.layernorm_affine_f8 if f8 else ops.layernorm_affine_q8 if q8 else
+        fuse_qn = (self.fuse_cross_qnorm and self.quant is None and ops.gemm_ssq_planes(B * L, C, C) == Hh and ops.flash_attn_qnorm_ok(Hh, c.text_len))
+        fold3 = (self.fold_layernorm and fuse_qn and premod and xs.is_contiguous() and ops.gemm_stats_planes(B * L, C, C, fs) == C // 128
+                 and ops.gemm_lnfold_ssq_planes(B * L, C, C) == Hh)
+        if fold3:
+            _, stats3 = ops.gemm_gate_res_stats(att.view(B, L, C), sa.o.weight, sa.o.bias, xs, xs, e0, 2, L, fs, tag="gemm_o")
+        else:
+            self._lin(att.view(B, L, C), pk, "o", sa.o.weight, sa.o.bias, ops.EPI_BIAS_GATE_RES, out=xs, res=xs, e=e0,
+                      mod=mod, gate_idx=2, rows_per_batch=L, frame_len=fs)
+        xn = None if fold3 else (ops.layernorm_affine_mx if mx else ops.layernorm_affine_mx6 if m6 else ops.layernorm_affine_mx4 if m4 else ops.layernorm_affine_f8 if f8 else ops.layernorm_affine_q8 if q8 else
               ops.layernorm_affine)(xs, blk.norm3.weight, blk.norm3.bias, c.eps)
-        fuse_qn = (self.fuse_cross_qnorm and self.quant is None and ops.gemm_ssq_planes(B * L, C, C) == Hh and ops.flash_attn_qnorm_ok(Hh, c.text_len))
-        if fuse_qn:
+        if fold3:
+            qraw, ssq = ops.gemm_lnfold_ssq(xs, self._lnfold_norm3(i), stats3, c.eps, tag="gemm_cq_ssq")
+        elif fuse_qn:
             qraw, ssq = ops.gemm_ssq(xn, ca.q.weight, ca.q.bias, tag="gemm_cq_ssq")
         else:
             qc = ops.rmsnorm(self._lin(xn, pk, "cq", ca.q.weight, ca.q.bias), ca.norm_q.weight, c.eps)
diff --git a/longlive_amd/ops.py b/longlive_amd/ops.py
--- a/longlive_amd/ops.py
+++ b/longlive_amd/ops.py
@@ -311,6 +311,70 @@
     t0 = _t0(tag)
     _lib.check(lib.ll_gemm_bf16_ssq(x.data_ptr(), w.data_ptr(), bias.data_ptr(), out.data_ptr(), ssq.data_ptr(), M, N, K, K, N, _stream()),
                "ll_gemm_bf16_ssq")
+    _t1(tag, t0, 2.0 * M * N * K)
+    return out, ssq
+
+
+def lnfold_premod(w, a, t, bias):
+    _chk(w, "w"); _chk(bias, "bias"); _chk(a, "a", torch.float32); _chk(t, "t", torch.float32)
+    N, K = w.shape
+    assert a.numel() == K and t.numel() == K and bias.numel() == N
+    wp = torch.empty_like(w)
+    sv = torch.empty(N, dtype=torch.float32, device=w.device)
+    cv = torch.empty(N, dtype=torch.float32, device=w.device)
+    _lib.check(_lib.load().ll_lnfold_premod(w.data_ptr(), a.data_ptr(), t.data_ptr(), bias.data_ptr(), wp.data_ptr(), sv.data_ptr(),
+                                            cv.data_ptr(), N, K, _stream()), "ll_lnfold_premod")
+    return wp, sv, cv
+
+
+def gemm_stats_planes(M: int, N: int, K: int, frame_len: int) -> int:
+    return int(_lib.load().ll_gemm_stats_planes(M, N, K, frame_len))
+
+
+def gemm_gate_res_stats(x, w, bias, out, res, e, gate_idx: int, rows_per_batch: int, frame_len: int, tag: str = "gemm"):
+    _chk(x, "x"); _chk(w, "w"); _chk(bias, "bias"); _chk(out, "out"); _chk(res, "res"); _chk(e, "e")
+    K = x.shape[-1]
+    M = x.numel() // K
+    N = w.shape[0]
+    nmod = e.shape[-2]
+    assert w.shape == (N, K) and bias.numel() == N and out.numel() == M * N and res.numel() == M * N
+    assert e.shape[-1] == N and e.numel() == (M // frame_len) * nmod * N, (e.shape, M, frame_len)
+    planes = gemm_stats_planes(M, N, K, frame_len)
+    if planes == 0:
+        raise RuntimeError(f"gemm_gate_res_stats: {M} x {N} x {K} is not covered by the generated kernel (use gemm)")
+    stats = torch.empty(2, planes, M, dtype=torch.float32, device=x.device)
+    lib = _lib.load()
+    t0 = _t0(tag)
+    _lib.check(lib.ll_gemm_bf16_gate_res_stats(x.data_ptr(), w.data_ptr(), bias.data_ptr(), out.data_ptr(), stats.data_ptr(), M, N, K, K, N,
+                                               res.data_ptr(), e.data_ptr(), nmod, gate_idx, rows_per_batch, frame_len, _stream()),
+               "ll_gemm_bf16_gate_res_stats")
+    _t1(tag, t0, 2.0 * M * N * K)
+    return out, stats
+
+
+def gemm_lnfold_ssq_planes(M: int, N: int, K: int) -> int:
+    return int(_lib.load().ll_gemm_lnfold_ssq_planes(M, N, K))
+
+
+def gemm_lnfold_ssq(x, premod, stats, eps: float, out=None, tag: str = "gemm"):
+    wp, sv, cv = premod
+    _chk(x, "x"); _chk(wp, "wp"); _chk(sv, "s", torch.float32); _chk(cv, "c", torch.float32); _chk(stats, "stats", torch.float32)
+    K = x.shape[-1]
+    M = x.numel() // K
+    N = wp.shape[0]
+    assert wp.shape == (N, K) and sv.numel() == N and cv.numel() == N and stats.shape == (2, K // 128, M), (wp.shape, stats.shape, M)
+    if out is None:
+        out = torch.empty(*x.shape[:-1], N, dtype=bf16, device=x.device)
+    _chk(out, "out")
+    assert out.numel() == M * N
+    planes = gemm_lnfold_ssq_planes(M, N, K)
+    if planes == 0:
+        raise RuntimeError(f"gemm_lnfold_ssq: {M} x {N} x {K} is not covered by the generated kernel (use layernorm_affine + gemm_ssq)")
+    ssq = torch.empty(planes, M, dtype=torch.float32, device=x.device)
+    lib = _lib.load()
+    t0 = _t0(tag)
+    _lib.check(lib.ll_gemm_lnfold_ssq(x.data_ptr(), wp.data_ptr(), sv.data_ptr(), cv.data_ptr(), stats.data_ptr(), eps, out.data_ptr(),
+                                      ssq.data_ptr(), M, N, K, N, _stream()), "ll_gemm_lnfold_ssq")
     _t1(tag, t0, 2.0 * M * N * K)
     return out, ssq
 
```

New measurement: 92.30, median of 6. No clear change (+0.7%).
